# mbdriscoll/indigo

Hardware: AMD Instinct MI355X
Metric: SENSE AHA evals/sec (256^3 x 8-coil non-Cartesian) (higher is better)
Workload: dtype complex64 (f32)

## Files before the change

include/indigo_hip.h:

```cpp
#ifndef INDIGO_HIP_H
#define INDIGO_HIP_H

#include <stddef.h>
#include <stdint.h>

#ifdef __cplusplus
extern "C" {
#endif

#define IG_ABI_VERSION 1

#define IG_OK            0
#define IG_ERR_HIP       1
#define IG_ERR_ARG       2
#define IG_ERR_NODEVICE  3
#define IG_ERR_UNSUPPORTED 4
#define IG_ERR_NOMEM     5

#define IG_H2D 1
#define IG_D2H 2
#define IG_D2D 3

typedef struct ig_ctx   ig_ctx;
typedef struct ig_fft   ig_fft;
// ... 68 lines not shown
int  ig_csoft_c64(ig_ctx* ctx, int64_t n0, int64_t n1, int64_t n2, int64_t c0, int64_t c1, int64_t c2, int64_t ncols,
                  float tau, void* x, int64_t ldx);
int  ig_grad3_c64(ig_ctx* ctx, int64_t n0, int64_t n1, int64_t n2, int64_t ncols, const void* x, int64_t ldx,
                  float alpha_re, float alpha_im, float beta_re, float beta_im, void* y, int64_t ldy);
int  ig_grad3h_c64(ig_ctx* ctx, int64_t n0, int64_t n1, int64_t n2, int64_t ncols, const void* u, int64_t ldu,
                   float alpha_re, float alpha_im, float beta_re, float beta_im, void* y, int64_t ldy);
int  ig_tv_dual_c64(ig_ctx* ctx, int64_t n0, int64_t n1, int64_t n2, int64_t ncols, const void* xn, int64_t ldxn,
                    const void* xo, int64_t ldxo, float sigma, float mu, void* u, int64_t ldu);
int  ig_grad4_c64(ig_ctx* ctx, int64_t n0, int64_t n1, int64_t n2, int64_t nt, const void* x, int64_t ldx,
                  float alpha_re, float alpha_im, float beta_re, float beta_im, void* y, int64_t ldy);
int  ig_grad4h_c64(ig_ctx* ctx, int64_t n0, int64_t n1, int64_t n2, int64_t nt, const void* u, int64_t ldu,
                   float alpha_re, float alpha_im, float beta_re, float beta_im, void* y, int64_t ldy);
int  ig_tv4_dual_c64(ig_ctx* ctx, int64_t n0, int64_t n1, int64_t n2, int64_t nt, const void* xn, int64_t ldxn,
                     const void* xo, int64_t ldxo, float sigma, float mu, float mu_t, void* u, int64_t ldu);
int  ig_llr_svt_c64(ig_ctx* ctx, int64_t n0, int64_t n1, int64_t n2, int64_t nt, int64_t b0, int64_t b1, int64_t b2,
                    int64_t s0, int64_t s1, int64_t s2, float tau, void* x, int64_t ldx);
int  ig_llr_nuc_c64(ig_ctx* ctx, int64_t n0, int64_t n1, int64_t n2, int64_t nt, int64_t b0, int64_t b1, int64_t b2,
                    int64_t s0, int64_t s1, int64_t s2, const void* x, int64_t ldx, float* nuc);
int  ig_basis_c64(ig_ctx* ctx, int64_t n, int64_t nk, int64_t nt, const void* phi, int64_t ldphi, int adjoint,
                  const void* x, int64_t ldx, float alpha_re, float alpha_im, float beta_re, float beta_im,
                  void* y, int64_t ldy);
int  ig_psf_mix_c64(ig_ctx* ctx, int64_t n, int64_t nc, int64_t nk, const float* kern, const void* x, int64_t ldx,
                    void* y, int64_t ldy, int64_t sg, int64_t sc);
int  ig_coil_maps_c64(ig_ctx* ctx, int64_t n, int64_t nc, int64_t nm, const void* maps, int adjoint, const void* x,
                      float alpha_re, float alpha_im, float beta_re, float beta_im, void* y, int64_t ldi, int64_t sg, int64_t sc);

int  ig_ccsrmm(ig_ctx* ctx, int adjoint, int exwrite,
               int64_t M, int64_t K, int64_t N, int64_t nnz,
               float alpha_re, float alpha_im,
               const void* vals, const int32_t* colind, const int32_t* rowptr,
               const void* X, int64_t ldx,
               float beta_re, float beta_im,
               void* Y, int64_t ldy);

int  ig_ccsrmm_t(ig_ctx* ctx,
                 int64_t M, int64_t K, int64_t N, int64_t nnz,
                 float alpha_re, float alpha_im,
                 const void* vals_t, const int32_t* colind_t, const int32_t* rowptr_t,
                 const void* X, int64_t ldx,
                 float beta_re, float beta_im,
                 void* Y, int64_t ldy);

int  ig_ccsrmm_t_grid(ig_ctx* ctx,
                      int64_t M, int64_t K, int64_t N, int64_t nnz,
                      float alpha_re, float alpha_im,
                      const void* vals_t, const int32_t* colind_t, const int32_t* rowptr_t,
                      const void* X, int64_t ldx,
                      float beta_re, float beta_im,
                      void* Y, int64_t ldy,
                      const int16_t* support, int64_t n0, int64_t nm, const int32_t* xrow_perm);

int  ig_ccsrmm_il(ig_ctx* ctx,
                  int64_t M, int64_t K, int64_t N, int64_t nnz,
                  float alpha_re, float alpha_im,
                  const void* vals, const int32_t* colind, const int32_t* rowptr,
                  const void* X_il,
                  float beta_re, float beta_im,
                  void* Y, int64_t ldy);
int  ig_ccsrmm_il_rw(ig_ctx* ctx,
                     int64_t M, int64_t K, int64_t N, int64_t nnz,
                     float alpha_re, float alpha_im,
                     const void* vals, const float* vals_re, const int32_t* colind, const int32_t* rowptr,
                     const void* X_il,
                     float beta_re, float beta_im,
                     void* Y, int64_t ldy);
int  ig_ccsrmm_t_grid_il(ig_ctx* ctx,
                         int64_t M, int64_t K, int64_t N, int64_t nnz,
                         float alpha_re, float alpha_im,
                         const void* vals_t, const int32_t* colind_t, const int32_t* rowptr_t,
                         const void* X, int64_t ldx,
                         void* Y_il,
                         const int16_t* support, int64_t n0, int64_t nm);

int  ig_grid_bricks_count(int64_t M, const int32_t* rowptr, const int32_t* colind, int64_t n0, int64_t nm, int64_t ns,
                          int bm, int bs, int unit, int32_t* brick_entries);
int  ig_grid_bricks_fill(int64_t M, const int32_t* rowptr, const int32_t* colind, const void* vals, int64_t n0, int64_t nm,
                         int64_t ns, int bm, int bs, int unit, const int64_t* brick_ptr, void* entries,
                         uint32_t* round_rows);
int  ig_ccsrmm_t_bricks(ig_ctx* ctx, int64_t M, int64_t K, int64_t N, float alpha_re, float alpha_im,
                        const void* entries, const uint32_t* round_rows, const void* X, int64_t ldx, void* Y_il,
                        const int16_t* support, int64_t n0, int64_t nm, int bm, int bs, const int32_t* tasks, int64_t ntasks,
                        const int32_t* brick_table, const int32_t* shared_bricks, int64_t nshared, int support_tile, int support_zwords,
                        int entry_words);

int  ig_grid_slots_build(int64_t nbricks, const int64_t* brick_ptr, const void* entries12, const uint32_t* entry_rows, int ncell,
                         void* entries16, int32_t* brick_slots, int32_t* slot_ptr, int64_t* nslots);
int  ig_ccsrmm_t_slots(ig_ctx* ctx, int64_t M, int64_t K, int64_t N, float alpha_re, float alpha_im,
                       const void* entries16, const int32_t* slot_ptr, const void* X, int64_t ldx, void* Y_il,
                       const int16_t* support, int64_t n0, int64_t nm, int bm, int bs, const int32_t* tasks, int64_t ntasks,
                       const int32_t* brick_table, const int32_t* shared_bricks, int64_t nshared, int support_tile, int support_zwords,
                       int entry_words );

int  ig_grid_gather_sep(ig_ctx* ctx, int64_t M, int64_t NC, int tw, const void* records, int64_t rec_stride, const void* X_il,
                        int64_t n0, int64_t nm, int64_t ns, float alpha_re, float alpha_im, float beta_re, float beta_im,
                        void* Y, int64_t ldy, const uint32_t* group_order);
int  ig_grid_gather_sep_group(int64_t NC, int tw);

int  ig_grid_shares_count(int64_t M, const uint32_t* records, int tw, int64_t n0, int64_t nm, int64_t ns, int bm, int bs, int32_t* brick_shares);
int  ig_grid_shares_fill(int64_t M, const uint32_t* records, int tw, int64_t n0, int64_t nm, int64_t ns, int bm, int bs,
                         const int64_t* brick_ptr, uint32_t* shares);
int  ig_grid_scatter_sep(ig_ctx* ctx, int64_t M, int64_t NC, int tw, void* records, int64_t rec_stride, const void* shares, const void* X, int64_t ldx,
                         void* Y_il, int64_t n0, int64_t nm, int64_t ns, int bm, int bs, const int32_t* tasks, int64_t ntasks,
                         const int32_t* brick_table, const int32_t* shared_table, int64_t nshared, int support_tile,
                         float alpha_re, float alpha_im);

int  ig_ccsrmm_t_bricks_wide(ig_ctx* ctx, int64_t M, int64_t K, float alpha_re, float alpha_im,
                             const void* entries, const uint32_t* entry_rows, const void* X, int64_t ldx, void* Y, int64_t ldy,
                             const int32_t* tasks, int64_t ntasks, const int32_t* brick_table, const uint32_t* owned_tiles);
int  ig_ccsrmm_t_bricks_wide_grid(ig_ctx* ctx, int64_t M, int64_t K, float alpha_re, float alpha_im,
                                  const void* entries, const uint32_t* entry_rows, const void* X, int64_t ldx, void* Y, int64_t ldy,
                                  const int32_t* tasks, int64_t ntasks, const int32_t* brick_table, const uint32_t* owned_tiles,
                                  int64_t n0, int64_t nm, int bm, int bs,
                                  int entry_words );

int  ig_ccsrmm_rowperm(ig_ctx* ctx, int64_t M, int64_t K, int64_t N, int64_t nnz,
                       float alpha_re, float alpha_im,
                       const void* vals, const int32_t* colind, const int32_t* rowptr,
                       const void* X, int64_t ldx,
                       float beta_re, float beta_im,
                       void* Y, int64_t ldy,
                       const int32_t* yrow_perm);

int  ig_ccsrmm_xrows(ig_ctx* ctx, int64_t M, int64_t K, int64_t N, int64_t nnz,
                     float alpha_re, float alpha_im,
                     const void* vals, const int32_t* colind_c, const int32_t* rowptr,
                     const void* X, int64_t ldx,
                     float beta_re, float beta_im,
                     void* Y, int64_t ldy,
                     const int32_t* xrows, int64_t nxrows);

int  ig_csr_runs_build(int64_t M, int64_t K, const int32_t* rowptr, const int32_t* colind, const void* vals,
                       int32_t* run_dptr, uint32_t* dcols, void* entries, int* all_real);
int  ig_ccsrmm_xrows_runs(ig_ctx* ctx, int64_t M, int64_t K, int64_t nnz, float alpha_re, float alpha_im, const int32_t* rowptr,
                          const int32_t* run_dptr, const uint32_t* dcols, const void* entries, int all_real,
                          const int32_t* run_order ,
                          const void* X, int64_t ldx, float beta_re, float beta_im, void* Y, int64_t ldy,
                          const int32_t* xrows, int64_t nxrows);

int  ig_csr_inspect(const int32_t* rowptr, const int32_t* colind, int64_t M, int64_t K,
                    int64_t* nzrow, int64_t* nzcol, int* exwrite);

int  ig_csr_transpose(int64_t M, int64_t K, int64_t nnz,
                      const int32_t* rowptr, const int32_t* colind, const void* vals,
                      int32_t* rowptr_t, int32_t* colind_t, void* vals_t);

int  ig_conemm(ig_ctx* ctx, int64_t M, int64_t K, int64_t N, float alpha_re, float alpha_im,
               const void* X, int64_t ldx, float beta_re, float beta_im, void* Y, int64_t ldy);
int  ig_cdiamm(ig_ctx* ctx, int adjoint, int64_t M, int64_t K, int64_t N, int64_t ndiag, const int32_t* offsets,
               const void* data, int64_t ld_data, float alpha_re, float alpha_im, const void* X, int64_t ldx,
               float beta_re, float beta_im, void* Y, int64_t ldy);
int  ig_cgemm(ig_ctx* ctx, int adjoint, int right, int64_t rows_m, int64_t cols_m, int64_t p,
              float alpha_re, float alpha_im, const void* M, int64_t ldm, const void* X, int64_t ldx,
              float beta_re, float beta_im, void* Y, int64_t ldy);

int  ig_interp3_count(int64_t m, const int64_t* N, double width, const double* coord, int32_t* rowptr);
int  ig_interp3_fill(int64_t m, const int64_t* N, double width, const double* table, int64_t ntable,
                     const double* coord, const int32_t* rowptr, int32_t* colind, float* weights, int grid_order);
int  ig_interp3_fill_modulated(int64_t m, const int64_t* N, double width, const double* table, int64_t ntable,
                               const double* coord, const int32_t* rowptr, int32_t* colind, void* values, int grid_order,
                               const double* phase_x, const double* phase_y, const double* phase_z, double scale);
int  ig_interp3_sep_words(int tw);
int  ig_interp3_sep(int64_t m, const int64_t* N, double width, const double* table, int64_t ntable, const double* coord,
                    int grid_order, const double* sign_x, const double* sign_y, const double* sign_z, double scale,
                    int tw, uint32_t* records);
int  ig_grid_support(int64_t nnz, const int32_t* colind, int64_t n0, int64_t n1, int64_t n2, int tile, int zw_in, int zw_out, int16_t* table);

int  ig_fft_plan(ig_ctx* ctx, int rank, const int64_t* dims, int64_t batch,
                 ig_fft** plan, size_t* workspace_bytes);
int  ig_fft_exec(ig_fft* plan, const void* x, void* y, int direction ,
                 void* workspace );
int  ig_fft_describe(ig_fft* plan, char* buf, size_t len);
int  ig_fft_inplace_workspace(ig_fft* plan, size_t* bytes);

int  ig_fft_plan_padded(ig_ctx* ctx, const int64_t* dims, const int64_t* box_lo, const int64_t* box_dims,
                        int64_t batch, int grid_layout, ig_fft** plan, size_t* workspace_bytes);
int  ig_fft_set_support_tile(ig_fft* plan, int tile);
int  ig_fft_set_axis_shift(ig_fft* plan, int axis, int64_t shift);
int64_t ig_fft_zc_size(const int64_t* dims, const int64_t* box_dims, int64_t coils, int64_t piece_bytes);
int64_t ig_fft_zc_offset(const int64_t* dims, const int64_t* box_dims, int64_t coils, int64_t piece_bytes, int64_t kx, int64_t ky, int64_t z, int64_t coil);
int  ig_fft_support_words(int64_t n2, int* zw_in, int* zw_out);
int  ig_fft_padded_axis_kind(int64_t n, int* kind);
int  ig_fft_exec_padded(ig_fft* plan, const void* x, int64_t x_bstride, const void* w, void* y, void* workspace,
                        const int16_t* support);
int  ig_fft_exec_cropped(ig_fft* plan, const void* y, const void* w, void* x, int64_t x_bstride, void* workspace,
                         const int16_t* support);
int  ig_fft_exec_cropped_sum(ig_fft* plan, const void* y, const void* w, void* x, void* workspace,
                             const int16_t* support);
// ... 25 lines not shown
```

indigo_amd/_lib.py:

```python
import ctypes
import os
import sys
from ctypes import (POINTER, c_char_p, c_double, c_float, c_int, c_int32, c_int64,
                    c_size_t, c_void_p)

_HERE = os.path.dirname(os.path.abspath(__file__))
_LIB = None

IG_OK = 0
IG_H2D, IG_D2H, IG_D2D = 1, 2, 3

PROTOTYPES = {
    "ig_abi_version":     (c_int, []),
    "ig_device_count":    (c_int, [POINTER(c_int)]),
    "ig_init":            (c_int, [c_int, POINTER(c_void_p)]),
    "ig_init_on_stream":  (c_int, [c_int, c_void_p, POINTER(c_void_p)]),
    "ig_destroy":         (None,  [c_void_p]),
    "ig_last_error":      (c_char_p, [c_void_p]),
    "ig_sync":            (c_int, [c_void_p]),
    "ig_stream":          (c_void_p, [c_void_p]),
    "ig_device_name":     (c_int, [c_void_p, c_char_p, c_size_t]),
    "ig_mem_info":        (c_int, [c_void_p, POINTER(c_size_t), POINTER(c_size_t)]),
    "ig_set_option":      (c_int, [c_void_p, c_char_p, c_int64]),
    "ig_library_bytes":   (c_int, [c_void_p, POINTER(c_size_t)]),
    "ig_malloc":          (c_int, [c_void_p, c_size_t, POINTER(c_void_p)]),
    "ig_free":            (c_int, [c_void_p, c_void_p]),
    "ig_probe_placement": (c_int, [c_void_p, c_void_p, c_size_t, POINTER(c_double)]),
    "ig_memset0":         (c_int, [c_void_p, c_void_p, c_size_t]),
    "ig_copy2d":          (c_int, [c_void_p, c_void_p, c_size_t, c_void_p, c_size_t, c_size_t, c_size_t, c_int]),
    "ig_event_create":    (c_int, [c_void_p, POINTER(c_void_p)]),
    "ig_event_record":    (c_int, [c_void_p]),
    "ig_event_elapsed_ms": (c_int, [c_void_p, c_void_p, POINTER(c_float)]),
    "ig_event_destroy":   (c_int, [c_void_p]),
    "ig_graph_begin":     (c_int, [c_void_p]),
    "ig_graph_end":       (c_int, [c_void_p, POINTER(c_void_p)]),
    "ig_graph_abort":     (c_int, [c_void_p]),
    "ig_graph_launch":    (c_int, [c_void_p]),
    "ig_graph_destroy":   (c_int, [c_void_p]),
    "ig_prof_enable":     (c_int, [c_void_p, c_int]),
    "ig_prof_report":     (c_int, [c_void_p, c_char_p, c_size_t]),
    "ig_caxpby":          (c_int, [c_void_p, c_int64, c_float, c_float, c_void_p, c_float, c_float, c_void_p]),
    "ig_cscal":           (c_int, [c_void_p, c_int64, c_float, c_float, c_void_p]),
    "ig_cdotc":           (c_int, [c_void_p, c_int64, c_void_p, c_void_p, POINTER(c_double)]),
    "ig_scnrm2sq":        (c_int, [c_void_p, c_int64, c_void_p, POINTER(c_double)]),
    "ig_cmax":            (c_int, [c_void_p, c_int64, c_float, c_void_p]),
    "ig_scalars":         (c_int, [c_void_p, POINTER(c_void_p), POINTER(c_int)]),
    "ig_cdotc_dev":       (c_int, [c_void_p, c_int64, c_void_p, c_void_p, c_void_p]),
    "ig_scnrm2sq_dev":    (c_int, [c_void_p, c_int64, c_void_p, c_void_p]),
    "ig_scalar_ratio":    (c_int, [c_void_p, c_void_p, c_void_p, c_void_p, c_double]),
    "ig_scalar_ratio_gated": (c_int, [c_void_p, c_void_p, c_void_p, c_void_p, c_double, c_void_p, c_void_p, c_double]),
    "ig_scalar_copy":     (c_int, [c_void_p, c_void_p, c_void_p, c_int64]),
    "ig_scalar_read":     (c_int, [c_void_p, c_void_p, c_int64, c_void_p]),
    "ig_cg_dot":          (c_int, [c_void_p, c_int64, c_void_p, c_void_p, c_float]),
    "ig_cg_step_r":       (c_int, [c_void_p, c_int64, c_void_p, c_void_p, c_void_p, c_void_p, c_double, c_void_p]),
    "ig_cg_step_xp":      (c_int, [c_void_p, c_int64, c_void_p, c_void_p, c_void_p, c_void_p, c_void_p, c_void_p, c_void_p, c_void_p]),
    "ig_caxpby_dev":      (c_int, [c_void_p, c_int64, c_void_p, c_float, c_void_p, c_void_p, c_float, c_void_p]),
    "ig_csum_cols":       (c_int, [c_void_p, c_int64, c_int64, c_void_p, c_int64, c_float, c_float, c_float, c_float, c_void_p]),
    "ig_csum_il":         (c_int, [c_void_p, c_int64, c_int64, c_void_p, c_float, c_float, c_float, c_float, c_void_p]),
    "ig_permute3_c64":    (c_int, [c_void_p, c_int64, c_int64, c_int64, c_void_p, c_int64, c_void_p, c_int64,
                                   c_float, c_float, c_float, c_float, c_void_p, c_int64]),
    "ig_dwt3_c64":        (c_int, [c_void_p, c_int64, c_int64, c_int64, c_int, c_int, c_int, c_int64, c_void_p, c_int64,
                                   c_float, c_float, c_float, c_float, c_void_p, c_int64]),
    "ig_csoft_c64":       (c_int, [c_void_p, c_int64, c_int64, c_int64, c_int64, c_int64, c_int64, c_int64, c_float,
                                   c_void_p, c_int64]),
    "ig_grad3_c64":       (c_int, [c_void_p, c_int64, c_int64, c_int64, c_int64, c_void_p, c_int64,
                                   c_float, c_float, c_float, c_float, c_void_p, c_int64]),
    "ig_grad3h_c64":      (c_int, [c_void_p, c_int64, c_int64, c_int64, c_int64, c_void_p, c_int64,
                                   c_float, c_float, c_float, c_float, c_void_p, c_int64]),
    "ig_tv_dual_c64":     (c_int, [c_void_p, c_int64, c_int64, c_int64, c_int64, c_void_p, c_int64, c_void_p, c_int64,
                                   c_float, c_float, c_void_p, c_int64]),
    "ig_grad4_c64":       (c_int, [c_void_p, c_int64, c_int64, c_int64, c_int64, c_void_p, c_int64,
                                   c_float, c_float, c_float, c_float, c_void_p, c_int64]),
    "ig_grad4h_c64":      (c_int, [c_void_p, c_int64, c_int64, c_int64, c_int64, c_void_p, c_int64,
                                   c_float, c_float, c_float, c_float, c_void_p, c_int64]),
    "ig_tv4_dual_c64":    (c_int, [c_void_p, c_int64, c_int64, c_int64, c_int64, c_void_p, c_int64, c_void_p, c_int64,
                                   c_float, c_float, c_float, c_void_p, c_int64]),
    "ig_llr_svt_c64":     (c_int, [c_void_p, c_int64, c_int64, c_int64, c_int64, c_int64, c_int64, c_int64, c_int64, c_int64, c_int64,
                                   c_float, c_void_p, c_int64]),
    "ig_llr_nuc_c64":     (c_int, [c_void_p, c_int64, c_int64, c_int64, c_int64, c_int64, c_int64, c_int64, c_int64, c_int64, c_int64,
                                   c_void_p, c_int64, c_void_p]),
    "ig_basis_c64":       (c_int, [c_void_p, c_int64, c_int64, c_int64, c_void_p, c_int64, c_int, c_void_p, c_int64,
                                   c_float, c_float, c_float, c_float, c_void_p, c_int64]),
    "ig_psf_mix_c64":     (c_int, [c_void_p, c_int64, c_int64, c_int64, c_void_p, c_void_p, c_int64, c_void_p, c_int64, c_int64, c_int64]),
    "ig_coil_maps_c64":   (c_int, [c_void_p, c_int64, c_int64, c_int64, c_void_p, c_int, c_void_p,
                                   c_float, c_float, c_float, c_float, c_void_p, c_int64, c_int64, c_int64]),
    "ig_ccsrmm_il":      (c_int, [c_void_p, c_int64, c_int64, c_int64, c_int64,
                                   c_float, c_float, c_void_p, c_void_p, c_void_p,
                                   c_void_p, c_float, c_float, c_void_p, c_int64]),
    "ig_ccsrmm_il_rw":    (c_int, [c_void_p, c_int64, c_int64, c_int64, c_int64,
                                   c_float, c_float, c_void_p, c_void_p, c_void_p, c_void_p,
                                   c_void_p, c_float, c_float, c_void_p, c_int64]),
    "ig_ccsrmm_t_grid_il": (c_int, [c_void_p, c_int64, c_int64, c_int64, c_int64,
                                    c_float, c_float, c_void_p, c_void_p, c_void_p,
                                    c_void_p, c_int64, c_void_p,
                                    c_void_p, c_int64, c_int64]),
    "ig_grid_bricks_count": (c_int, [c_int64, c_void_p, c_void_p, c_int64, c_int64, c_int64, c_int, c_int, c_int, c_void_p]),
    "ig_grid_bricks_fill": (c_int, [c_int64, c_void_p, c_void_p, c_void_p, c_int64, c_int64, c_int64, c_int, c_int, c_int, c_void_p, c_void_p, c_void_p]),
    "ig_ccsrmm_t_bricks": (c_int, [c_void_p, c_int64, c_int64, c_int64, c_float, c_float, c_void_p, c_void_p,
                                   c_void_p, c_int64, c_void_p, c_void_p, c_int64, c_int64, c_int, c_int, c_void_p, c_int64,
                                   c_void_p, c_void_p, c_int64, c_int, c_int, c_int]),
    "ig_ccsrmm":          (c_int, [c_void_p, c_int, c_int, c_int64, c_int64, c_int64, c_int64,
                                   c_float, c_float, c_void_p, c_void_p, c_void_p,
                                   c_void_p, c_int64, c_float, c_float, c_void_p, c_int64]),
    "ig_ccsrmm_t":        (c_int, [c_void_p, c_int64, c_int64, c_int64, c_int64,
                                   c_float, c_float, c_void_p, c_void_p, c_void_p,
                                   c_void_p, c_int64, c_float, c_float, c_void_p, c_int64]),
    "ig_ccsrmm_t_grid":   (c_int, [c_void_p, c_int64, c_int64, c_int64, c_int64,
                                   c_float, c_float, c_void_p, c_void_p, c_void_p,
                                   c_void_p, c_int64, c_float, c_float, c_void_p, c_int64,
                                   c_void_p, c_int64, c_int64, c_void_p]),
    "ig_grid_slots_build": (c_int, [c_int64, c_void_p, c_void_p, c_void_p, c_int, c_void_p, c_void_p, c_void_p, POINTER(c_int64)]),
    "ig_ccsrmm_t_slots":  (c_int, [c_void_p, c_int64, c_int64, c_int64, c_float, c_float, c_void_p, c_void_p, c_void_p, c_int64, c_void_p,
                                   c_void_p, c_int64, c_int64, c_int, c_int, c_void_p, c_int64, c_void_p, c_void_p, c_int64, c_int, c_int, c_int]),
    "ig_ccsrmm_t_bricks_wide": (c_int, [c_void_p, c_int64, c_int64, c_float, c_float, c_void_p, c_void_p, c_void_p, c_int64, c_void_p, c_int64,
                                        c_void_p, c_int64, c_void_p, c_void_p]),
    "ig_ccsrmm_t_bricks_wide_grid": (c_int, [c_void_p, c_int64, c_int64, c_float, c_float, c_void_p, c_void_p, c_void_p, c_int64, c_void_p, c_int64,
                                             c_void_p, c_int64, c_void_p, c_void_p, c_int64, c_int64, c_int, c_int, c_int]),
    "ig_fft_set_support_tile": (c_int, [c_void_p, c_int]),
    "ig_fft_set_axis_shift": (c_int, [c_void_p, c_int, c_int64]),
    "ig_csr_runs_build":  (c_int, [c_int64, c_int64, c_void_p, c_void_p, c_void_p, c_void_p, c_void_p, c_void_p, POINTER(c_int)]),
    "ig_ccsrmm_xrows_runs": (c_int, [c_void_p, c_int64, c_int64, c_int64, c_float, c_float, c_void_p, c_void_p, c_void_p, c_void_p, c_int, c_void_p,
                                     c_void_p, c_int64, c_float, c_float, c_void_p, c_int64, c_void_p, c_int64]),
    "ig_ccsrmm_xrows":    (c_int, [c_void_p, c_int64, c_int64, c_int64, c_int64,
                                   c_float, c_float, c_void_p, c_void_p, c_void_p,
                                   c_void_p, c_int64, c_float, c_float, c_void_p, c_int64, c_void_p, c_int64]),
    "ig_ccsrmm_rowperm":  (c_int, [c_void_p, c_int64, c_int64, c_int64, c_int64,
                                   c_float, c_float, c_void_p, c_void_p, c_void_p,
                                   c_void_p, c_int64, c_float, c_float, c_void_p, c_int64, c_void_p]),
    "ig_csr_inspect":     (c_int, [c_void_p, c_void_p, c_int64, c_int64,
                                   POINTER(c_int64), POINTER(c_int64), POINTER(c_int)]),
    "ig_csr_transpose":   (c_int, [c_int64, c_int64, c_int64, c_void_p, c_void_p, c_void_p,
                                   c_void_p, c_void_p, c_void_p]),
    "ig_conemm":          (c_int, [c_void_p, c_int64, c_int64, c_int64, c_float, c_float, c_void_p, c_int64, c_float, c_float, c_void_p, c_int64]),
    "ig_cdiamm":          (c_int, [c_void_p, c_int, c_int64, c_int64, c_int64, c_int64, c_void_p, c_void_p, c_int64,
                                   c_float, c_float, c_void_p, c_int64, c_float, c_float, c_void_p, c_int64]),
    "ig_cgemm":           (c_int, [c_void_p, c_int, c_int, c_int64, c_int64, c_int64, c_float, c_float, c_void_p, c_int64,
                                   c_void_p, c_int64, c_float, c_float, c_void_p, c_int64]),
    "ig_interp3_count":   (c_int, [c_int64, POINTER(c_int64), c_double, c_void_p, c_void_p]),
    "ig_interp3_fill":    (c_int, [c_int64, POINTER(c_int64), c_double, c_void_p, c_int64, c_void_p, c_void_p, c_void_p, c_void_p, c_int]),
    "ig_grid_support":    (c_int, [c_int64, c_void_p, c_int64, c_int64, c_int64, c_int, c_int, c_int, c_void_p]),
    "ig_fft_support_words": (c_int, [c_int64, POINTER(c_int), POINTER(c_int)]),
    "ig_fft_padded_axis_kind": (c_int, [c_int64, POINTER(c_int)]),
    "ig_fft_zc_size":     (c_int64, [POINTER(c_int64), POINTER(c_int64), c_int64, c_int64]),
    "ig_fft_zc_offset":   (c_int64, [POINTER(c_int64), POINTER(c_int64), c_int64, c_int64, c_int64, c_int64, c_int64, c_int64]),
    "ig_interp3_sep_words": (c_int, [c_int]),
    "ig_interp3_sep":     (c_int, [c_int64, POINTER(c_int64), c_double, c_void_p, c_int64, c_void_p, c_int, c_void_p, c_void_p, c_void_p, c_double,
                                   c_int, c_void_p]),
    "ig_grid_gather_sep": (c_int, [c_void_p, c_int64, c_int64, c_int, c_void_p, c_int64, c_void_p, c_int64, c_int64, c_int64, c_float, c_float, c_float, c_float,
                                   c_void_p, c_int64, c_void_p]),
    "ig_grid_gather_sep_group": (c_int, [c_int64, c_int]),
    "ig_grid_shares_count": (c_int, [c_int64, c_void_p, c_int, c_int64, c_int64, c_int64, c_int, c_int, c_void_p]),
    "ig_grid_shares_fill": (c_int, [c_int64, c_void_p, c_int, c_int64, c_int64, c_int64, c_int, c_int, c_void_p, c_void_p]),
    "ig_grid_scatter_sep": (c_int, [c_void_p, c_int64, c_int64, c_int, c_void_p, c_int64, c_void_p, c_void_p, c_int64, c_void_p, c_int64, c_int64, c_int64,
                                    c_int, c_int, c_void_p, c_int64, c_void_p, c_void_p, c_int64, c_int, c_float, c_float]),
    "ig_interp3_fill_modulated": (c_int, [c_int64, POINTER(c_int64), c_double, c_void_p, c_int64, c_void_p, c_void_p, c_void_p, c_void_p, c_int,
                                          c_void_p, c_void_p, c_void_p, c_double]),
    "ig_fft_plan":        (c_int, [c_void_p, c_int, POINTER(c_int64), c_int64, POINTER(c_void_p), POINTER(c_size_t)]),
    "ig_fft_exec":        (c_int, [c_void_p, c_void_p, c_void_p, c_int, c_void_p]),
    "ig_fft_describe":    (c_int, [c_void_p, c_char_p, c_size_t]),
    "ig_fft_inplace_workspace": (c_int, [c_void_p, POINTER(c_size_t)]),
    "ig_fft_destroy":     (c_int, [c_void_p]),
    "ig_fft_plan_padded": (c_int, [c_void_p, POINTER(c_int64), POINTER(c_int64), POINTER(c_int64), c_int64, c_int,
                                   POINTER(c_void_p), POINTER(c_size_t)]),
    "ig_fft_exec_padded": (c_int, [c_void_p, c_void_p, c_int64, c_void_p, c_void_p, c_void_p, c_void_p]),
    "ig_fft_exec_cropped": (c_int, [c_void_p, c_void_p, c_void_p, c_void_p, c_int64, c_void_p, c_void_p]),
    "ig_fft_exec_cropped_sum": (c_int, [c_void_p, c_void_p, c_void_p, c_void_p, c_void_p, c_void_p]),
    "ig_fft_exec_cropped_sum_slab": (c_int, [c_void_p, c_void_p, c_void_p, c_void_p, c_void_p, c_void_p, c_int, c_int64, c_int64]),
    "ig_fft_exec_cropped_slab": (c_int, [c_void_p, c_void_p, c_void_p, c_void_p, c_int64, c_void_p, c_void_p, c_int, c_int64, c_int64]),
    "ig_comm_preflight":  (c_int, []),
    "ig_comm_unique_id":  (c_int, [c_void_p]),
    "ig_comm_init_rank":  (c_int, [c_void_p, c_int, c_int, c_void_p, POINTER(c_void_p)]),
    "ig_comm_init_direct": (c_int, [c_void_p, c_int, c_int, c_char_p, c_size_t, c_double, POINTER(c_void_p)]),
    "ig_comm_info":       (c_int, [c_void_p, POINTER(c_int), POINTER(c_int), c_char_p, c_size_t]),
    "ig_allreduce_sum_f32": (c_int, [c_void_p, c_void_p, c_int64]),
    "ig_allreduce_sum_f32_side": (c_int, [c_void_p, c_void_p, c_int64]),
    "ig_comm_join":       (c_int, [c_void_p]),
    "ig_allreduce_max_f64_host": (c_int, [c_void_p, POINTER(c_double)]),
    "ig_allreduce_sum_f64_host": (c_int, [c_void_p, POINTER(c_double)]),
    "ig_comm_barrier":    (c_int, [c_void_p]),
    "ig_comm_destroy":    (c_int, [c_void_p]),
}


def lib_path():
    return os.environ.get("INDIGO_HIP_LIB") or os.path.join(_HERE, "lib", "libindigo_hip.so")


def lib():
    global _LIB
    if _LIB is not None:
        return _LIB
    path = lib_path()
    if not os.path.exists(path):
        raise RuntimeError(
            "indigo_amd: %s not found. Build it with `python -m indigo_amd.build` "
            "(needs hipcc); there is no CPU fallback." % path)
    if os.environ.get("INDIGO_HIP_WITH_TORCH", "0") == "1" and "torch" not in sys.modules:
        import torch
    handle = ctypes.CDLL(path)
    for name, (res, args) in PROTOTYPES.items():
        fn = getattr(handle, name)
        fn.restype = res
        fn.argtypes = args
    if handle.ig_abi_version() != 1:
        raise RuntimeError("indigo_amd: ABI version mismatch in %s" % path)
    _LIB = handle
    return _LIB


def last_error(ctx=None):
    msg = lib().ig_last_error(ctx)
    return msg.decode("utf-8", "replace") if msg else ""


def cplx(v):
    v = complex(v)
    return ctypes.c_float(v.real), ctypes.c_float(v.imag)


def check(rc, ctx=None, what=""):
    if rc != IG_OK:
        raise RuntimeError("%s failed (status %d): %s" % (what or "libindigo_hip call", rc, last_error(ctx)))


def device_count():
    n = c_int(0)
    lib().ig_device_count(ctypes.byref(n))
    return n.value
```

indigo_amd/analyses.py:

```python
from contextlib import contextmanager

import numpy as np

from indigo_amd.transforms import Visitor
from indigo_amd import operators as op


class Memusage(Visitor):

    def measure(self, node, ncols=1):
        self._seen = set()
        self._base = 0
        self._live = [0]
        self._cols = [ncols]
        self._peak = 0
        self.visit(node)
        return self._base + self._peak

    @contextmanager
    def _push(self, stack, value):
        stack.append(value)
        try:
            yield
        finally:
            stack.pop()

    def _ncols(self):
        return int(np.prod(self._cols, dtype=np.int64))

    def _round(self, nbytes):
        return nbytes

    def visit(self, node):
        self._peak = max(self._peak, sum(self._live))
        if isinstance(node, op.ZpadFFTMaps) and id(node) not in self._seen:
            self._seen.add(id(node))
            self._base += node.maps_bytes()
        if isinstance(node, (op.Product, op.UnscaledFFT, op.ZpadFFT, op.HeadRows)):
            with self._push(self._live, self._round(node._mem_usage(self._ncols()))):
                self._peak = max(self._peak, sum(self._live))
                self.generic_visit(node)
        elif isinstance(node, op.ToeplitzNormal):
            if id(node) not in self._seen:
                self._seen.add(id(node))
                self._base += node.kernel_bytes()
            with self._push(self._live, self._round(node._mem_usage(self._ncols()))):
                self._peak = max(self._peak, sum(self._live))
        elif isinstance(node, op.Kron) and isinstance(node.left, op.Eye):
            with self._push(self._cols, node.left.shape[0]):
                self.visit(node.right)
        elif isinstance(node, op.SpMatrix):
            if id(node) not in self._seen:
                self._seen.add(id(node))
                self._base += (node.shape[0] + 1) * 4 + node.nnz * 4 + node.nnz * 8
        elif isinstance(node, (op.DenseMatrix, op.FrameBasis, op.CoilMaps)):
            if id(node) not in self._seen:
                self._seen.add(id(node))
                self._base += node._matrix.nbytes
        else:
            self.generic_visit(node)


class ScratchUsage(Memusage):

    def measure(self, node, ncols=1):
        super().measure(node, ncols)
        return self._peak // 8

    def _round(self, nbytes):
        elems = (nbytes + 7) // 8
        return (elems + 31) // 32 * 32 * 8


class TreeHasOp(Visitor):
    def __init__(self, op_classes):
        self._op_classes = tuple(op_classes)

    def search(self, node):
        self._found = False
        self.visit(node)
        return self._found

    def visit(self, node):
        if isinstance(node, self._op_classes):
            self._found = True
        self.generic_visit(node)
```

indigo_amd/backends/backend.py:

```python
import logging
from contextlib import contextmanager

import numpy as np
import scipy.sparse as spp

import indigo_amd.operators as op

log = logging.getLogger(__name__)
_C64 = np.dtype('complex64')


WAVELETS = {
    'haar': (2 ** -0.5, 2 ** -0.5),
    'db2': (0.48296291314453416, 0.8365163037378079, 0.22414386804201339, -0.12940952255126037),
    'db4': (0.23037781330889645, 0.7148465705529156, 0.630880767929859, -0.027983769416859594,
            -0.18703481171909306, 0.03084138183556063, 0.032883011666885176, -0.010597401785069018),
}
WAVELET_IDS = {'haar': 0, 'db2': 1, 'db4': 2}
DWT_MAX_AXIS = 1024


def dwt_plan(dims, wavelet, levels):
    taps = len(WAVELETS[wavelet])
    c = [int(n) for n in dims]
# ... 154 lines not shown
                return None
            dup = self._backend.zero_array(self.shape, self.dtype, name=name)
            dup._copy(self)
            return dup

        @classmethod
        def to_device(cls, backend, arr, name=''):
            arr_f = np.require(arr, requirements='F')
            d_arr = cls(backend, arr.shape, arr.dtype, name=name)
            d_arr.copy_from(arr_f)
            return d_arr

        def __setitem__(self, slc, other):
            assert isinstance(slc, slice) and not (slc.start or slc.stop), "dndarray setitem cant slice"
            self._copy(other)

        def __del__(self):
            if getattr(self, '_own', False) and hasattr(self, '_arr'):
                self._memory.pop(id(self), None)
                try:
                    self._free()
                except Exception:
                    pass

        def __getitem__(self, slc):
            raise NotImplementedError()

        def _copy_from(self, arr):
            raise NotImplementedError()

        def _copy_to(self, arr):
            raise NotImplementedError()

        def _copy(self, d_arr):
            raise NotImplementedError()

        def _malloc(self, shape, dtype):
            raise NotImplementedError()

        def _free(self):
            raise NotImplementedError()

        def _zero(self):
            raise NotImplementedError()

    def copy_array(self, arr, name=''):
        return self.dndarray.to_device(self, arr, name=name)

    def empty_array(self, shape, dtype, name=''):
        return self.dndarray(self, shape, dtype, name=name)

    def zero_array(self, shape, dtype, name=''):
        d_arr = self.empty_array(shape, dtype, name=name)
        d_arr._zero()
        return d_arr

    def zeros_like(self, other, name=''):
        return self.zero_array(other.shape, other.dtype, name=name)

    def rand_array(self, shape, dtype=_C64, name='', seed=None):
        rng = np.random.default_rng(seed)
        x = rng.random(shape) + 1j * rng.random(shape)
        x = np.require(x, dtype=_C64, requirements='F')
        return self.copy_array(x, name=name)

    def get_max_threads(self):
        return 1

    def barrier(self):
        pass

    def mem_usage(self):
        total = 0
        rows = []
        for name, shape, dtype in list(self.dndarray._memory.values()):
            n = int(np.prod(shape, dtype=np.int64)) * dtype.itemsize
            rows.append((n, name, shape, dtype))
            total += n
        log.info("Memory report:")
        for n, name, shape, dtype in sorted(rows, key=lambda r: r[0]):
            if n > 1e6:
                log.info("  %40s: % 3.0f MB, %20s, %15s", name, n / 1e6, shape, dtype)
        return total

    def reserve_scratch(self, nelems):
        self._scratch = self.empty_array((max(int(nelems), 1),), _C64, name='scratch')
        self._scratch_pos = 0

    @contextmanager
    def scratch(self, shape=None, nbytes=None):
        assert not (shape is not None and nbytes is not None), \
            "Specify either shape or nbytes to backend.scratch()."
        if nbytes is not None:
            shape = (int(nbytes) // _C64.itemsize,)
        size = int(np.prod(shape, dtype=np.int64))
        arena = getattr(self, '_scratch', None)
        if arena is not None and self._scratch_pos + size > arena.size:
            log.warning("scratch arena too small (wanted %d elements at offset %d of %d); allocating dynamically",
                        size, self._scratch_pos, arena.size)
            arena = None
        if arena is not None:
            pos = self._scratch_pos
            mem = arena[pos:pos + size].reshape(tuple(shape))
            bump = (size + 31) // 32 * 32
            self._scratch_pos += bump
            try:
                yield mem
            finally:
                self._scratch_pos -= bump
        else:
            mem = self.zero_array(tuple(shape), dtype=_C64, name='scratch(dynamic)')
            yield mem
            del mem

    def SpMatrix(self, M=None, **kwargs):
        assert (M is not None and spp.issparse(M)) or kwargs.get('struct') is not None
        return op.SpMatrix(self, M, **kwargs)

    def DenseMatrix(self, M, **kwargs):
        assert isinstance(M, np.ndarray) and M.ndim == 2
        return op.DenseMatrix(self, M, **kwargs)

    def Diag(self, v, **kwargs):
        v = np.require(v, requirements='F')
        if v.ndim > 1:
            v = v.flatten(order='A')
        dtype = kwargs.pop('dtype', _C64)
        if np.dtype(dtype) == _C64:
            from indigo_amd.structured import DiagS
            return self.SpMatrix(struct=DiagS(v.size, [('vec', v.astype(_C64))]), **kwargs)
        return self.SpMatrix(spp.diags(v, offsets=0).astype(dtype), **kwargs)

    def Adjoint(self, A, **kwargs):
        return op.Adjoint(self, A, **kwargs)

    def KronI(self, c, B, **kwargs):
        return op.Kron(self, self.Eye(c), B, **kwargs)

    def Kron(self, A, B, **kwargs):
        return op.Kron(self, A, B, **kwargs)

    def BlockDiag(self, Ms, **kwargs):
        return op.BlockDiag(self, *Ms, **kwargs)

    def VStack(self, Ms, **kwargs):
        return op.VStack(self, *Ms, **kwargs)

    def HStack(self, Ms, **kwargs):
        return op.HStack(self, *Ms, **kwargs)

    def UnscaledFFT(self, shape, dtype=_C64, **kwargs):
        return op.UnscaledFFT(self, shape, dtype=dtype, **kwargs)

    def Eye(self, n, dtype=_C64, **kwargs):
        return op.Eye(self, n, dtype=dtype, **kwargs)

    def ZpadFFT(self, grid_shape, box_shape, weights, **kwargs):
        return op.ZpadFFT(self, grid_shape, box_shape, weights, **kwargs)

    def One(self, shape, dtype=_C64, **kwargs):
        return op.One(self, shape, dtype=dtype, **kwargs)

    def FFT(self, shape, dtype=_C64, **kwargs):
        n = int(np.prod(shape))
        if np.dtype(dtype) == _C64:
            from indigo_amd.structured import DiagS
            c = (np.ones(1, dtype=dtype) / np.sqrt(n))[0]
            return self.SpMatrix(struct=DiagS(n, [('const', c)]), name='scale') * self.UnscaledFFT(shape, dtype, **kwargs)
        s = np.ones(n, order='F', dtype=dtype) / np.sqrt(n)
        return self.Diag(s, name='scale') * self.UnscaledFFT(shape, dtype, **kwargs)

    @staticmethod
    def fftc_mod_phases(ft_shape):
        return [(np.arange(n) - (n // 2) / 2.0) * ((n // 2) / n) for n in ft_shape]

    @staticmethod
    def fftc_mod(ft_shape, dtype=_C64):
        phase = 0
        for i, ph in enumerate(Backend.fftc_mod_phases(ft_shape)):
            phase = phase + ph.reshape([-1 if j == i else 1 for j in range(len(ft_shape))])
        return np.exp(1j * 2.0 * np.pi * phase).astype(dtype)

    def FFTc(self, ft_shape, dtype=_C64, normalize=True, **kwargs):
        if np.dtype(dtype) == _C64:
            from indigo_amd.structured import DiagS, SepPhase
            M = self.SpMatrix(struct=DiagS(int(np.prod(ft_shape)), [('sep', SepPhase(ft_shape, self.fftc_mod_phases(ft_shape)))]), name='mod')
        else:
            M = self.Diag(self.fftc_mod(ft_shape, dtype), name='mod')
        F = self.FFT(ft_shape, dtype=dtype, **kwargs) if normalize else self.UnscaledFFT(ft_shape, dtype=dtype, **kwargs)
        return M * F * M

    @staticmethod
    def zpad_rows(M, N, mode='center'):
        if mode == 'center':
            slc = tuple(slice(m // 2 + int(np.ceil(-n / 2)), m // 2 + int(np.ceil(n / 2))) for m, n in zip(M, N))
        elif mode == 'edge':
            slc = tuple(slice(n) for n in N)
        else:
            raise ValueError("unknown zpad mode %r" % mode)
        x = np.arange(int(np.prod(M)), dtype=np.int64).reshape(M, order='F')
        return x[slc].flatten(order='F')

    def Zpad(self, M, N, mode='center', dtype=_C64, **kwargs):
        rows = self.zpad_rows(M, N, mode)
        cols = np.arange(rows.size)
        if np.dtype(dtype) == _C64:
            from indigo_amd.structured import SelectS
            return self.SpMatrix(struct=SelectS((int(np.prod(M)), int(np.prod(N))), rows, cols, np.ones(rows.size, dtype=_C64)), **kwargs)
        mat = spp.coo_matrix((np.ones(rows.size), (rows, cols)), shape=(int(np.prod(M)), int(np.prod(N))), dtype=dtype)
        return self.SpMatrix(mat, **kwargs)

    def Crop(self, M, N, dtype=_C64, **kwargs):
        return self.Zpad(N, M, dtype=dtype, **kwargs).H

    def AxisPermute(self, dims, perm, **kwargs):
        return op.AxisPermute(self, dims, perm, **kwargs)

# ... 297 lines not shown
        w = int(width) if (interleaved and width is not None) else C
        K2 = kern.size // n
        K = int(round(np.sqrt(K2)))
        assert n >= 1 and C >= 1 and w >= C and K * K * n == kern.size, (kern.shape, n)
        rows = n * w
        assert x.size == rows * K and y.size == rows * K, (x.shape, y.shape, n, w, K)
        P = self.psf_unpack(kern.to_host(), n, K)
        shape = (w, n, K) if interleaved else (n, w, K)
        v = x.to_host().reshape(shape, order='F').astype(np.complex128)
        out = y.to_host().reshape(shape, order='F').copy()
        if interleaved:
            out[:C] = np.einsum('gab,cgb->cga', P, v[:C]).astype(_C64)
        else:
            out[:] = np.einsum('gab,gcb->gca', P, v).astype(_C64)
        y.copy_from(np.asfortranarray(out.reshape(y.shape, order='F')))

    def ToeplitzNormal(self, dims, maps, kern, K, **kwargs):
        return op.ToeplitzNormal(self, dims, maps, kern, K, **kwargs)

    def supports_padded_fft(self, grid, ncoils=None):
        return False

    def ccsrmm(self, y, A_shape, A_indx, A_ptr, A_vals, x, alpha=1, beta=0, adjoint=False, exwrite=False):
        raise NotImplementedError()

    def cdiamm(self, y, shape, offsets, data, x, alpha=1.0, beta=0.0, adjoint=True):
        raise NotImplementedError()

    def onemm(self, y, x, alpha=1, beta=0):
        raise NotImplementedError()

    def cgemm(self, y, M, x, alpha, beta, forward):
        raise NotImplementedError()

    def csymm(self, y, M, x, alpha, beta, left=True):
        raise NotImplementedError()

    def max(self, val, arr):
        raise NotImplementedError()

    def inspect(self, csr):
        counts = np.bincount(csr.indices, minlength=csr.shape[1])
        nzrow = int(np.count_nonzero(np.diff(csr.indptr)))
        return nzrow, int(np.count_nonzero(counts)), bool(counts.max(initial=0) <= 1)

    class csr_matrix(object):
        _index_base = 0

        def __init__(self, backend, A, name='mat'):
            if not spp.isspmatrix_csr(A):
                A = A.tocsr()
            A = self._type_correct(A)
            assert A.nnz < 2 ** 31 and max(A.shape) < 2 ** 31, "int32 CSR indices"
            self._backend = backend
            self._name = name
            self.shape = tuple(int(s) for s in A.shape)
            self.dtype = A.dtype
            self.rowPtrs = backend.copy_array(A.indptr.astype(np.int32) + self._index_base, name=name + ".rowPtrs")
            self.colInds = backend.copy_array(A.indices.astype(np.int32) + self._index_base, name=name + ".colInds")
            self.values = backend.copy_array(A.data, name=name + ".data")
            nzrow, nzcol, self._exwrite = backend.inspect(A)
            self._row_frac = nzrow / A.shape[0] if A.shape[0] else 1.0
            self._col_frac = nzcol / A.shape[1] if A.shape[1] else 1.0
            self._grid_il = False

        @staticmethod
        def _check_panels(y, x, vals):
            assert x.dtype == _C64, "Bad dtype: expected complex64, got %s" % x.dtype
            assert y.dtype == _C64, "Bad dtype: expected complex64, got %s" % y.dtype
            assert vals.dtype == _C64

        def forward(self, y, x, alpha=1, beta=0):
            self._check_panels(y, x, self.values)
            il = {'x_il': True} if self._grid_il else {}
            self._backend.ccsrmm(y, self.shape, self.colInds, self.rowPtrs, self.values,
                                 x, alpha=alpha, beta=beta, adjoint=False, exwrite=True, **il)

        def adjoint(self, y, x, alpha=1, beta=0):
            self._check_panels(y, x, self.values)
            il = {'y_il': True} if self._grid_il else {}
            self._backend.ccsrmm(y, self.shape, self.colInds, self.rowPtrs, self.values,
                                 x, alpha=alpha, beta=beta, adjoint=True, exwrite=self._exwrite, **il)

        def set_grid_interleaved(self, flag=True):
            self._grid_il = bool(flag)

        def set_grid_support(self, table, n0, nm, zw=16):
            pass

        def set_grid_bricks(self, n0, nm, ns, ncols=8, bm=2, bs=2, chunk=4096, run=4096):
            pass

        def set_row_order(self, perm):
            pass

        @property
        def nbytes(self):
            return self.rowPtrs.nbytes + self.colInds.nbytes + self.values.nbytes

        @property
        def nnz(self):
            return self.values.size

        def _type_correct(self, A):
            return A.astype(_C64)

    class dia_matrix(object):

        def __init__(self, backend, A, name='mat'):
            assert isinstance(A, spp.dia_matrix)
            A = A.astype(_C64)
            self._backend = backend
            self.data = backend.copy_array(np.asfortranarray(A.data.T), name=name + ".data")
            self.offsets = backend.copy_array(A.offsets.astype(np.int32), name=name + ".offsets")
            self.shape = tuple(int(s) for s in A.shape)
            self.dtype = A.dtype
            self._row_frac = 1
            self._col_frac = 1
            self._exwrite = False

        def forward(self, y, x, alpha=1, beta=0):
            self._backend.cdiamm(y, self.shape, self.offsets, self.data, x, alpha=alpha, beta=beta, adjoint=False)

        def adjoint(self, y, x, alpha=1, beta=0):
            self._backend.cdiamm(y, self.shape, self.offsets, self.data, x, alpha=alpha, beta=beta, adjoint=True)

        @property
        def nbytes(self):
            return self.offsets.nbytes + self.data.nbytes

        @property
        def nnz(self):
            return self.data.size

    def cg(self, A, b_h, x_h, lamda=0.0, tol=1e-10, maxiter=100, team=None):
        in_place = isinstance(x_h, self.dndarray)
        x = x_h if in_place else self.copy_array(x_h, name='x')
        resid = b_h.copy(name='b') if isinstance(b_h, self.dndarray) else self.copy_array(b_h, name='b')
        q = x.copy()

        def shifted(dst, src):
            A.eval(dst, src)
            if lamda:
                self.axpby(1, dst, lamda, src)

        shifted(q, x)
        self.axpby(1, resid, -1, q)
        d = resid.copy(name='p')
        rho = rho0 = self.pnorm2(resid, team)
        trail = []
        for it in range(maxiter):
            shifted(q, d)
            step = rho / self.pdot(d, q, team)
            self.axpby(1, x, step, d)
            self.axpby(1, resid, -step, q)
            rho, rho_old = self.pnorm2(resid, team), rho
            self.axpby(rho / rho_old, d, 1, resid)
            trail.append(float(np.sqrt(rho / rho0)))
            log.info("iter %d, residual %g", it, trail[-1])
            if trail[-1] < tol:
                log.info("cg reached tolerance")
                break
        else:
            log.info("cg reached maxiter")
        if not in_place:
            x.copy_to(x_h)
# ... 62 lines not shown
```

indigo_amd/backends/hip.py:

```python
import ctypes
import logging
import os

import numpy as np

from indigo_amd import _lib
from indigo_amd._lib import cplx as _cplx
from indigo_amd.backends.backend import WAVELET_IDS, Backend
from indigo_amd.grid_formats import brick_tasks, weights_are_real

log = logging.getLogger(__name__)
_C64 = np.dtype('complex64')


class HipBackend(Backend):

    def __init__(self, device_id=0, stream=None):
        super().__init__(device_id)
        self._L = _lib.lib()
        ctx = ctypes.c_void_p()
        if stream is None:
            rc = self._L.ig_init(int(device_id), ctypes.byref(ctx))
        else:
            rc = self._L.ig_init_on_stream(int(device_id), ctypes.c_void_p(stream), ctypes.byref(ctx))
        _lib.check(rc, None, "ig_init")
        self._ctx = ctx
        self.device_id = int(device_id)
        self._plans = dict()
        self.adjoint_policy = 'transpose'
        self._placement_log = []
        self.tuning = dict(placement_candidates=3, placement_min_bytes=1 << 31, placement_window_gb=24, placement_window_allocs=3, fold_odd_axes=True, real_gridding=True, gather_order=True, cg_graph=False, bricks=(4, 8), slots=(1, 2), slot_shape=(4, 4, 256, 64), support_tile={8: 4, 4: 8}, brick_shape={8: (2, 2, 4096, 4096), 4: (2, 4, 4096, 4096)}, xrows=True, runs=True, wide_bricks=True,
                           wide_brick_shape=(2, 2), wide_task_shape=(8192, 2048),
                           separable=True, sep_gather=True, sep_scatter=True, shares=(4, 8), shares_min_tw=6, share_shape={8: (4, 4, 128, 1024), 4: (4, 4, 128, 1024)})

    def __del__(self):
        try:
            for entry in getattr(self, '_plans', {}).values():
                self._L.ig_fft_destroy(entry[0])
            if getattr(self, '_ctx', None):
                self._L.ig_destroy(self._ctx)
                self._ctx = None
        except Exception:
            pass

    def _check(self, rc, what):
        if rc != 0:
            _lib.check(rc, self._ctx, what)

    def barrier(self):
        self._check(self._L.ig_sync(self._ctx), "ig_sync")

    @property
    def stream(self):
        return self._L.ig_stream(self._ctx) or 0

    def device_name(self):
        buf = ctypes.create_string_buffer(256)
        self._check(self._L.ig_device_name(self._ctx, buf, 256), "ig_device_name")
        return buf.value.decode()

    def set_option(self, name, value):
        self._check(self._L.ig_set_option(self._ctx, name.encode(), int(value)), "ig_set_option(%s)" % name)
        for entry in self._plans.values():
            self._L.ig_fft_destroy(entry[0])
        self._plans = dict()

    def mem_usage(self):
        own = ctypes.c_size_t()
        self._check(self._L.ig_library_bytes(self._ctx, ctypes.byref(own)), "ig_library_bytes")
        return super().mem_usage() + own.value

    def mem_info(self):
        free, total = ctypes.c_size_t(), ctypes.c_size_t()
        self._check(self._L.ig_mem_info(self._ctx, ctypes.byref(free), ctypes.byref(total)), "ig_mem_info")
        return free.value, total.value

    def event(self):
        ev = ctypes.c_void_p()
        self._check(self._L.ig_event_create(self._ctx, ctypes.byref(ev)), "ig_event_create")
        return ev

    def record(self, ev):
        self._check(self._L.ig_event_record(ev), "ig_event_record")

    def elapsed_ms(self, start, stop):
        ms = ctypes.c_float()
        self._check(self._L.ig_event_elapsed_ms(start, stop, ctypes.byref(ms)), "ig_event_elapsed_ms")
        return ms.value

    def event_destroy(self, ev):
        self._L.ig_event_destroy(ev)

    def profile(self, on=True):
        self._check(self._L.ig_prof_enable(self._ctx, 1 if on else 0), "ig_prof_enable")
        self._prof_on = bool(on)

    def profile_report(self):
        buf = ctypes.create_string_buffer(1 << 16)
        self._check(self._L.ig_prof_report(self._ctx, buf, len(buf)), "ig_prof_report")
        out = {}
        for line in buf.value.decode().splitlines():
            name, n, ms, nbytes = line.split()
            out[name] = dict(launches=int(n), total_ms=float(ms), avg_ms=float(ms) / max(int(n), 1), bytes=float(nbytes))
        return out

    class dndarray(Backend.dndarray):

        def _malloc(self, shape, dtype):
            b = self._backend
            if self.nbytes >= int(b.tuning.get('placement_min_bytes', 1 << 31)):
                slack = int(b.tuning.get('placement_window_gb', 0))
                if slack > 0:
                    ptr = self._malloc_window(slack)
                    if ptr is not None:
                        return ptr
                ncand = int(b.tuning.get('placement_candidates', 1))
                if ncand > 1:
                    return self._malloc_best_placed(ncand)
            ptr = ctypes.c_void_p()
            b._check(b._L.ig_malloc(b._ctx, self.nbytes, ctypes.byref(ptr)), "ig_malloc(%d bytes)" % self.nbytes)
            return ptr.value

        def _malloc_window(self, slack_gb):
            b = self._backend
            GBs = 1 << 30
            nalloc = max(1, int(b.tuning.get('placement_window_allocs', 3)))
            worst = b.tuning.get('placement_pick') == 'worst'
            cands = []
            try:
                for _ in range(nalloc):
                    free, total = ctypes.c_size_t(), ctypes.c_size_t()
                    need = (self.nbytes + (slack_gb + 4) * GBs) if not cands else 2 * (self.nbytes + slack_gb * GBs)
                    if b._L.ig_mem_info(b._ctx, ctypes.byref(free), ctypes.byref(total)) != 0 or free.value < need:
                        break
                    base = ctypes.c_void_p()
                    if b._L.ig_malloc(b._ctx, self.nbytes + slack_gb * GBs, ctypes.byref(base)) != 0:
                        break
                    cands.append([None, base.value, 0, []])
                    times = []
                    for off in range(slack_gb + 1):
                        ms = ctypes.c_double(0.0)
                        b._check(b._L.ig_probe_placement(b._ctx, ctypes.c_void_p(base.value + off * GBs), self.nbytes, ctypes.byref(ms)), "ig_probe_placement")
                        times.append(ms.value)
                    if len(cands) == 1:
# ... 767 lines not shown
```

indigo_amd/backends/hip_csr.py:

```python
import logging

import numpy as np

from indigo_amd import _lib, grid_formats
from indigo_amd._lib import cplx as _cplx
from indigo_amd.backends.backend import Backend

log = logging.getLogger(__name__)
_C64 = np.dtype('complex64')

_BRICK_ARRAYS = dict(tasks=".brickTasks", table=".brickTable", entries=".brickEntries", rounds=".brickRoundRows", shared=".sharedBricks")
_SLOT_ARRAYS = dict(tasks=".slotTasks", table=".slotTable", entries=".slotEntries", slot_ptr=".slotPtr", shared=".slotSharedBricks")
_SHARE_ARRAYS = dict(tasks=".shareTasks", table=".shareTable", shares=".shares", shared=".shareSharedBricks")
_WIDE_ARRAYS = dict(owned=".wideOwnedTiles", tasks=".wideTasks", table=".wideTable", entries=".wideEntries", rows=".wideEntryRows")
_RUN_ARRAYS = dict(order=".runOrder", dptr=".runPtr", dcols=".runCols", entries=".runEntries")


def _ptr(a):
    return None if a is None else a._arr


class csr_matrix(Backend.csr_matrix):

    def __init__(self, backend, A, name='mat'):
# ... 183 lines not shown
        if self._perm is None and 16 <= ncols <= 64 and self._col_frac <= 0.6 and self.values.size >= self.shape[1] and t['xrows']:
            sub = self._touched()
            return 'xrows_runs' if ncols == 64 and t.get('runs', True) and sub[0].size * 512 < 2 ** 32 and self._runs(sub) is not None else 'xrows'
        return 'csr' if self._perm is None else 'rowperm'

    def adjoint_route(self, ncols, beta, y):
        b, perm = self._backend, self._perm
        scatter = perm is None and beta == 0 and y.contiguous
        shf = self._format('_shares', ncols, exact=True)
        if shf is not None and scatter and self._grid_il and shf['ntasks'] > 0 and b.tuning.get('sep_scatter', True):
            return 'shares'
        br = self._format('_bricks', ncols, exact=True)
        if br is not None and scatter and self._grid_il and ncols == br['ncols']:
            return 'bricks'
        sl = self._format('_slots', ncols, exact=True)
        if sl is not None and scatter and ncols == sl['ncols'] and sl['ntasks'] > 0:
            return 'slots'
        if (ncols == 64 and beta == 0 and perm is None and not self._grid_il and self.shape[1] % 16 == 0
                and self.shape[1] > 0 and self.shape[0] * 512 < 2 ** 31 and self.values.size >= self.shape[1] // 4
                and b.tuning['wide_bricks'] and self._wide_bricks() is not None):
            return 'wide'
        if self._grid_il:
            assert scatter, "interleaved panels: no row order, beta = 0"
            return 'gather_il'
        if perm is not None:
            assert not self._exwrite and b.adjoint_policy == 'transpose' and ncols <= 8, \
                "row-ordered matrices use the packed transposed gather"
        if (self._gather_support() is not None or perm is not None) and not self._exwrite and b.adjoint_policy == 'transpose':
            return 'gather_t_grid'
        return 'scatter' if self._exwrite or b.adjoint_policy != 'transpose' else 'gather_t'

    def _gather_support(self):
        return self._support if self._support_zw == 16 else None

    def _scatter_support(self, ncols, y):
        fine = self._format('_support_fine', ncols)
        tab, tile = fine if fine is not None else (self._support[0] if self._support is not None else None, 16)
        if tab is None:
            y._zero()
        return tab, tile

    def _call(self, kernel, *args):
        b = self._backend
        b._check(getattr(b._L, kernel)(b._ctx, *args), kernel)

    def _fwd_sep(self, y, x, alpha, beta):
        sep = self._sep
        order = self._gather_order(x.shape[1]) if self._backend.tuning.get('gather_order', True) else None
        self._call("ig_grid_gather_sep", self.shape[0], x.shape[1], sep['tw'], sep['records']._arr, sep['stride'], x._arr, *sep['dims'],
                   *_cplx(complex(alpha) * sep['gconst']), *_cplx(beta), y._arr, y._leading_dim, _ptr(order))

    def _fwd_il_rw(self, y, x, alpha, beta):
        self._call("ig_ccsrmm_il_rw", *self.shape, x.shape[1], self.values.size, *_cplx(alpha), self.values._arr, self._real_values()._arr,
                   self.colInds._arr, self.rowPtrs._arr, x._arr, *_cplx(beta), y._arr, y._leading_dim)

    def _fwd_il(self, y, x, alpha, beta):
        self._call("ig_ccsrmm_il", *self.shape, x.shape[1], self.values.size, *_cplx(alpha), self.values._arr, self.colInds._arr,
                   self.rowPtrs._arr, x._arr, *_cplx(beta), y._arr, y._leading_dim)

    def _fwd_xrows_runs(self, y, x, alpha, beta):
        sub, runs = self._xrows, self._runs_fmt
        self._call("ig_ccsrmm_xrows_runs", *self.shape, self.values.size, *_cplx(alpha), self.rowPtrs._arr, runs['dptr']._arr, runs['dcols']._arr,
                   runs['entries']._arr, runs['all_real'], _ptr(runs['order']), x._arr, x._leading_dim, *_cplx(beta), y._arr, y._leading_dim,
                   sub[0]._arr, sub[0].size)

    def _fwd_xrows(self, y, x, alpha, beta):
        sub = self._xrows
        self._call("ig_ccsrmm_xrows", *self.shape, x.shape[1], self.values.size, *_cplx(alpha), self.values._arr, sub[1]._arr, self.rowPtrs._arr,
                   x._arr, x._leading_dim, *_cplx(beta), y._arr, y._leading_dim, sub[0]._arr, sub[0].size)

    def _fwd_rowperm(self, y, x, alpha, beta):
        self._call("ig_ccsrmm_rowperm", *self.shape, x.shape[1], self.values.size, *_cplx(alpha), self.values._arr, self.colInds._arr,
                   self.rowPtrs._arr, x._arr, x._leading_dim, *_cplx(beta), y._arr, y._leading_dim, self._perm._arr)

    _FORWARD = dict(sep=_fwd_sep, il_rw=_fwd_il_rw, il=_fwd_il, xrows_runs=_fwd_xrows_runs, xrows=_fwd_xrows, rowperm=_fwd_rowperm,
                    csr=Backend.csr_matrix.forward)

    def forward(self, y, x, alpha=1, beta=0):
        if self._grid_il:
            assert self._perm is None and x.contiguous, "interleaved panels: no row order, contiguous grid panel"
        self._check_panels(y, x, self.values)
        self._FORWARD[self.forward_route(x.shape[1])](self, y, x, alpha, beta)

    def _adj_shares(self, y, x, alpha, beta):
        sep, shf = self._sep, self._format('_shares', x.shape[1], exact=True)
        self._scatter_support(x.shape[1], y)
        self._call("ig_grid_scatter_sep", self.shape[0], x.shape[1], sep['tw'], sep['recx']._arr, sep['stride_x'], shf['shares']._arr, x._arr,
                   x._leading_dim, y._arr, *sep['dims'], shf['bm'], shf['bs'], shf['tasks']._arr, shf['ntasks'], shf['table']._arr,
                   shf['shared']._arr, shf['nshared'], shf['tile'], *_cplx(complex(alpha) * np.conj(sep['gconst'])))

    def _adj_bricks(self, y, x, alpha, beta, kernel="ig_ccsrmm_t_bricks", which='_bricks', rows='rounds'):
        f = self._format(which, x.shape[1], exact=True)
        tab, tile = self._scatter_support(x.shape[1], y)
        self._call(kernel, *self.shape, x.shape[1], *_cplx(alpha), f['entries']._arr, f[rows]._arr, x._arr, x._leading_dim, y._arr, _ptr(tab),
                   f['n0'], f['nm'], f['bm'], f['bs'], f['tasks']._arr, f['ntasks'], f['table']._arr, f['shared']._arr, f['nshared'], tile,
                   self._support_zw, f['words'])

    def _adj_slots(self, y, x, alpha, beta):
        self._adj_bricks(y, x, alpha, beta, "ig_ccsrmm_t_slots", '_slots', 'slot_ptr')

    def _adj_wide(self, y, x, alpha, beta):
        wb = self._wide
        self._call("ig_ccsrmm_t_bricks_wide_grid", *self.shape, *_cplx(alpha), wb['entries']._arr, wb['rows']._arr, x._arr, x._leading_dim, y._arr,
                   y._leading_dim, wb['tasks']._arr, wb['ntasks'], wb['table']._arr, wb['owned']._arr, *wb['geom'], wb['words'])

    def _adj_gather_il(self, y, x, alpha, beta):
        pt, it, dt = self._transposed()
        tab, n0, nm = self._gather_support() or (None, 0, 0)
        self._call("ig_ccsrmm_t_grid_il", *self.shape, x.shape[1], dt.size, *_cplx(alpha), dt._arr, it._arr, pt._arr, x._arr, x._leading_dim,
                   y._arr, _ptr(tab), n0, nm)

    def _adj_gather_t(self, y, x, alpha, beta):
        pt, it, dt = self._transposed()
        self._backend.ccsrmm_t(y, self.shape, it, pt, dt, x, alpha=alpha, beta=beta, support=self._gather_support(), xperm=self._perm)

    def _adj_scatter(self, y, x, alpha, beta):
        self._backend.ccsrmm(y, self.shape, self.colInds, self.rowPtrs, self.values, x, alpha=alpha, beta=beta, adjoint=True, exwrite=self._exwrite)

    _ADJOINT = dict(shares=_adj_shares, bricks=_adj_bricks, slots=_adj_slots, wide=_adj_wide, gather_il=_adj_gather_il,
                    gather_t_grid=_adj_gather_t, scatter=_adj_scatter, gather_t=_adj_gather_t)

    def adjoint(self, y, x, alpha=1, beta=0):
        self._check_panels(y, x, self.values)
        self._ADJOINT[self.adjoint_route(x.shape[1], beta, y)](self, y, x, alpha, beta)
```

indigo_amd/csrc/ig_gridsep.hip:

```cpp
#include "ig_common.h"
#include <vector>
#include <thread>
#include <atomic>
#include <algorithm>
#include <cstring>

namespace {

constexpr int BLK = 256;
constexpr int WPB = BLK / 64;

__device__ __forceinline__ int64_t xcd_block(int64_t b, int64_t nb) {
    const int64_t q = nb >> 3, rem = nb & 7;
    const int64_t xcd = b & 7, idx = b >> 3;
    return (xcd < rem) ? xcd * (q + 1) + idx : rem * (q + 1) + (xcd - rem) * q + idx;
}

__host__ __device__ constexpr int sep_words(int tw) { return tw == 4 ? 16 : 32; }

template <int NC, int TW, int NBT, int CG>
__device__ __forceinline__ void gather_rows(float4& acc, const float4* __restrict__ X4, const uint32_t (&offm)[TW], const float (&w1)[TW],
                                            const float (&w2)[TW], float w0, int j2, int c2, int ns, uint32_t plane, int nc2u) {
#pragma unroll
    for (int c0 = 0; c0 < TW; c0 += CG) {
        if (c0 >= nc2u) break;
        float4 v[CG][NBT];
#pragma unroll
        for (int g = 0; g < CG; ++g) {
            int cc = c0 + g;
            cc = cc < c2 ? cc : c2 - 1;
            int js = j2 + cc;
            if (js >= ns) js -= ns;
            const uint32_t offs = (uint32_t)js * plane;
#pragma unroll
            for (int b = 0; b < NBT; ++b) v[g][b] = X4[(size_t)(offs + offm[b])];
        }
#pragma unroll
        for (int g = 0; g < CG; ++g) {
            const float ws = (c0 + g < c2) ? w0 * w2[c0 + g < TW ? c0 + g : 0] : 0.f;
#pragma unroll
            for (int b = 0; b < NBT; ++b) {
                const float w = ws * w1[b];
                acc.x = fmaf(w, v[g][b].x, acc.x); acc.y = fmaf(w, v[g][b].y, acc.y);
                acc.z = fmaf(w, v[g][b].z, acc.z); acc.w = fmaf(w, v[g][b].w, acc.w);
            }
        }
    }
}

template <int NC, int TW, int BMODE>
__global__ void __launch_bounds__(BLK)
k_grid_gather_sep(int64_t M, const uint32_t* __restrict__ rec, int rs , const float4* __restrict__ X4, int n0, int nm, int ns,
                  float2* __restrict__ Y, int64_t ldy, float2 alpha, float2 beta, const uint32_t* __restrict__ order) {
    constexpr int QL = NC / 2, XL = TW <= 4 ? 4 : 8, LPS = QL * XL, SPW = 64 / LPS;
    constexpr int CG = TW <= 4 ? 4 : 2;
    static_assert(LPS <= 64 && NC >= 2, "a sample's lanes fit a wave");
    const int lane = threadIdx.x & 63;
    const int q = lane % QL, i = (lane / QL) % XL, g = lane / LPS;
    int64_t blk = xcd_block(blockIdx.x, gridDim.x);
    if (order) { const uint32_t o = order[blk]; blk = o < gridDim.x ? (int64_t)o : blk; }
    const int64_t wave = blk * WPB + (threadIdx.x >> 6);
    const int64_t t = wave * SPW + g;
    const bool ok = t < M;
    const uint32_t* __restrict__ r = rec + (size_t)(ok ? t : M - 1) * (uint32_t)rs;
    const uint32_t h0 = r[3 * TW], h1 = r[3 * TW + 1];
    const int j0 = (int)(h0 & 0xffffu), j1 = (int)(h0 >> 16), j2 = (int)(h1 & 0xffffu);
    const int c0 = (int)((h1 >> 16) & 15u), c1 = (int)((h1 >> 20) & 15u), c2 = (int)((h1 >> 24) & 15u);
    const int iv = i < c0 ? i : c0 - 1;
    const float w0 = (i < c0 && ok) ? __uint_as_float(r[iv]) : 0.f;
    float w1[TW], w2[TW];
#pragma unroll
    for (int b = 0; b < TW; ++b) { w1[b] = b < c1 ? __uint_as_float(r[TW + b]) : 0.f; w2[b] = __uint_as_float(r[2 * TW + b]); }
    int jx = j0 + iv;
    if (jx >= n0) jx -= n0;
    uint32_t offm[TW];
#pragma unroll
    for (int b = 0; b < TW; ++b) {
        int jm = j1 + (b < c1 ? b : c1 - 1);
        if (jm >= nm) jm -= nm;
        offm[b] = ((uint32_t)jm * (uint32_t)n0 + (uint32_t)jx) * QL + q;
    }
    const uint32_t plane = (uint32_t)nm * (uint32_t)n0 * QL;
    int nc2u = 1;
#pragma unroll
    for (int v = TW; v > 1; --v)
        if (__builtin_amdgcn_ballot_w64(c2 >= v)) { nc2u = v; break; }
    float4 acc = make_float4(0.f, 0.f, 0.f, 0.f);
    if (__builtin_amdgcn_ballot_w64(c1 >= TW)) gather_rows<NC, TW, TW, CG>(acc, X4, offm, w1, w2, w0, j2, c2, ns, plane, nc2u);
    else                                       gather_rows<NC, TW, TW - 1, CG>(acc, X4, offm, w1, w2, w0, j2, c2, ns, plane, nc2u);
#pragma unroll
    for (int off = QL; off < LPS; off <<= 1) {
        acc.x += __shfl_xor(acc.x, off, 64); acc.y += __shfl_xor(acc.y, off, 64);
        acc.z += __shfl_xor(acc.z, off, 64); acc.w += __shfl_xor(acc.w, off, 64);
    }
    if (i == 0 && ok) {
        float2* y0 = Y + (int64_t)(2 * q) * ldy + t;
        float2* y1 = y0 + ldy;
        float2 o0 = cmul(alpha, make_float2(acc.x, acc.y)), o1 = cmul(alpha, make_float2(acc.z, acc.w));
        if (BMODE == 1) { cfma(o0, beta, *y0); cfma(o1, beta, *y1); }
        *y0 = o0;
        *y1 = o1;
    }
}

struct ShareTask { int32_t lo, hi, bt, nb_flags; };
struct ShareBrick { int32_t brick, end; uint32_t mask_lo, mask_hi; };

typedef float v16f_t __attribute__((ext_vector_type(16)));

template <bool SHARED, int NG, int XW>
__device__ __forceinline__ void mfma_flush(v16f_t (&acc)[NG], float* __restrict__ Yf, int64_t pt, uint64_t mask, float2 alpha, float sgn_ai, bool f_ok,
                                           int beta, int mn, int n0, int nm, int bm, int bs, int st_log2) {
    const int xs_log2 = 4 - st_log2;
    const int xseg = (4 * beta) >> st_log2;
#pragma unroll
    for (int g = 0; g < NG; ++g) {
        if (g < bs) {
#pragma unroll
            for (int b = 0; b < 4; ++b) {
                if (b < bm) {
                    float* dst = Yf + (pt + 4 * beta + (int64_t)n0 * (b + (int64_t)nm * g)) * XW + mn;
                    const bool mine = f_ok && ((mask >> (xseg + ((b + bm * g) << xs_log2))) & 1ull);
                    float o[4];
#pragma unroll
                    for (int r = 0; r < 4; ++r) {
                        const float v = acc[g][4 * b + r];
                        const float pv = __int_as_float(__builtin_amdgcn_update_dpp(0, __float_as_int(v), 0xB1, 0xf, 0xf, false));
                        o[r] = fmaf(alpha.x, v, sgn_ai * pv);
                    }
                    if (mine) {
                        if (SHARED)
                            asm volatile("global_atomic_add_f32 %0, %1, off\n\tglobal_atomic_add_f32 %0, %2, off offset:%5\n\t"
                                         "global_atomic_add_f32 %0, %3, off offset:%6\n\tglobal_atomic_add_f32 %0, %4, off offset:%7"
                                         :: "v"(dst), "v"(o[0]), "v"(o[1]), "v"(o[2]), "v"(o[3]), "i"(XW * 4), "i"(2 * XW * 4), "i"(3 * XW * 4) : "memory");
                        else
                            asm volatile("global_store_dword %0, %1, off\n\tglobal_store_dword %0, %2, off offset:%5\n\t"
                                         "global_store_dword %0, %3, off offset:%6\n\tglobal_store_dword %0, %4, off offset:%7"
                                         :: "v"(dst), "v"(o[0]), "v"(o[1]), "v"(o[2]), "v"(o[3]), "i"(XW * 4), "i"(2 * XW * 4), "i"(3 * XW * 4) : "memory");
                    }
                    __builtin_amdgcn_sched_barrier(0);
                }
            }
        }
#pragma unroll
        for (int e = 0; e < 16; ++e) acc[g][e] = 0.f;
    }
}

template <int NC, int TW, int NG>
__global__ void __launch_bounds__(BLK, 3)
k_grid_scatter_mfma(const ShareTask* __restrict__ tasks, int ntasks, const ShareBrick* __restrict__ btab, const uint2* __restrict__ shares,
                    const uint32_t* __restrict__ recx, int rs ,
                    float* __restrict__ Yf, float2 alpha, int n0, int nm, int bm_log2, int bs_log2, int nbx, int nbm, int st_log2) {
    constexpr int RW = sep_words(TW), XW = 2 * NC, ZL = 3 * TW + 2;
    constexpr int PW = RW + 16;
    constexpr int G = 4, R = 16;
    static_assert(PW + TW + 6 <= 64 && XW <= 16 && NG == 4, "a ring slot holds record, panel row and the padded slow-axis weights");
    __shared__ uint32_t ring_all[WPB][R][64];
    __shared__ uint2 hdr_all[WPB][128];
    const int tid = threadIdx.x, lane = tid & 63;
    const int wv = __builtin_amdgcn_readfirstlane(tid >> 6);
    const int task = blockIdx.x * WPB + wv;
    if (task >= ntasks) return;
    const ShareTask tk = tasks[task];
    const int nb = tk.nb_flags & 0xffff;
    const bool shared = (tk.nb_flags >> 16) & 1;
    const int nsh = tk.hi - tk.lo;
    const int bm = 1 << bm_log2, bs = 1 << bs_log2;
    const int beta = lane >> 4, mn = lane & 15;
    uint32_t* __restrict__ ring = &ring_all[wv][0][0];

    int my_end = 0x7fffffff;
    uint32_t my_mlo = 0xffffffffu, my_mhi = 0xffffffffu;
    int64_t my_pt = 0;
    if (lane < nb) {
        const ShareBrick br = btab[tk.bt + lane];
        if (!shared) my_end = br.end - tk.lo;
        my_mlo = br.mask_lo; my_mhi = br.mask_hi;
        const int bx = br.brick % nbx, bmi = (br.brick / nbx) % nbm, bsi = br.brick / (nbx * nbm);
        my_pt = (int64_t)bx * 16 + (int64_t)n0 * (((int64_t)bmi << bm_log2) + (int64_t)nm * ((int64_t)bsi << bs_log2));
    }
    v16f_t acc[NG];
#pragma unroll
    for (int g = 0; g < NG; ++g)
// ... 18 lines not shown
    auto load_batch = [&](int b) __attribute__((always_inline)) {
        const int idx = b * 64 + lane;
        return idx < nsh ? shp[idx] : make_uint2(0u, 0u);
    };
    {
        const uint2 b0 = load_batch(0), b1 = load_batch(1);
        hdrs[lane] = b0;
        hdrs[64 + lane] = b1;
    }
    uint2 sh_next = load_batch(2);
    int cb = 0;

    auto request = [&](uint32_t (&w)[G], int gi) __attribute__((always_inline)) {
#pragma unroll
        for (int k = 0; k < G; ++k) {
            const int sraw = G * gi + k;
            const int sc = sraw < nsh ? sraw : nsh - 1;
            const uint32_t t = (uint32_t)__builtin_amdgcn_readfirstlane((int)hdrs[sc & 127].x) & 0x0fffffffu;
            w[k] = lane_base[(size_t)t * (uint32_t)rs];
        }
    };
    auto stage = [&](const uint32_t (&w)[G], int gi) __attribute__((always_inline)) {
#pragma unroll
        for (int k = 0; k < G; ++k) ring[((G * gi + k) & (R - 1)) * 64 + lane] = w[k];
    };
    auto process = [&](int gi) __attribute__((always_inline)) {
        for (int k = 0; k < G; ++k) {
            const int s = G * gi + k;
            if (s >= nsh) break;
            if (s >= cur_end) {
                int ph, pl; uint32_t mlo, mhi;
                brick_of(ph, pl, mlo, mhi);
                mfma_flush<false, NG, XW>(acc, Yf, ((int64_t)ph << 32) | (uint32_t)pl, ((uint64_t)mhi << 32) | mlo, alpha, sgn_ai, f_ok, beta, mn, n0, nm, bm, bs, st_log2);
                ++cur;
                cur_end = __builtin_amdgcn_readlane(my_end, cur & 63);
            }
            const uint2 hd = hdrs[s & 127];
            const uint32_t geo = (uint32_t)__builtin_amdgcn_readfirstlane((int)hd.y), gmask = (uint32_t)__builtin_amdgcn_readfirstlane((int)hd.x) >> 28;
            const char* slot = reinterpret_cast<const char*>(ring) + (s & (R - 1)) * 256;
            const int ox4 = (int)(geo & 31u) * 4 - 32, om4 = (int)((geo >> 5) & 31u) * 4 - 32, os4 = (int)((geo >> 10) & 31u) * 4 - 32;
            const unsigned dx = (unsigned)(mn4 - ox4), db = (unsigned)(beta4 - om4);
            const float ax = __uint_as_float(*reinterpret_cast<const uint32_t*>(slot + (dx < (unsigned)(4 * TW) ? dx : (unsigned)(4 * ZL))));
            const float wm = __uint_as_float(*reinterpret_cast<const uint32_t*>(slot + (db - 4u * TW < (unsigned)(4 * TW) ? db : (unsigned)(4 * ZL))));
            const float xv = __uint_as_float(*reinterpret_cast<const uint32_t*>(slot + xv_off));
            const uint32_t* wsp = reinterpret_cast<const uint32_t*>(slot + (PW + 3) * 4 - os4);
            const float bmx = wm * xv;
#pragma unroll
            for (int g = 0; g < NG; ++g)
                if ((gmask >> g) & 1u)
                    acc[g] = __builtin_amdgcn_mfma_f32_16x16x1f32(ax, bmx * __uint_as_float(wsp[g]), acc[g], 0, 0, 0);
        }
    };

    const int ngroups = (nsh + G - 1) / G;
    uint32_t wa[G], wb[G];
    request(wa, 0);
    request(wb, 1);
    stage(wa, 0);
    for (int gi = 0; gi < ngroups; gi += 2) {
        if (((G * gi) >> 6) != cb) {
            ++cb;
            hdrs[((cb + 1) & 1) * 64 + lane] = sh_next;
            sh_next = load_batch(cb + 2);
        }
        request(wa, gi + 2);
        process(gi);
        stage(wb, gi + 1);
        request(wb, gi + 3);
        process(gi + 1);
        stage(wa, gi + 2);
    }
    {
        int ph, pl; uint32_t mlo, mhi;
        brick_of(ph, pl, mlo, mhi);
        const int64_t pt = ((int64_t)ph << 32) | (uint32_t)pl;
        const uint64_t mask = ((uint64_t)mhi << 32) | mlo;
        if (shared) mfma_flush<true, NG, XW>(acc, Yf, pt, mask, alpha, sgn_ai, f_ok, beta, mn, n0, nm, bm, bs, st_log2);
        else        mfma_flush<false, NG, XW>(acc, Yf, pt, mask, alpha, sgn_ai, f_ok, beta, mn, n0, nm, bm, bs, st_log2);
    }
}

template <int NC>
__global__ void __launch_bounds__(BLK)
k_sep_pack_recx(int64_t rows, const float2* __restrict__ X, int64_t ld, float2* __restrict__ recx2 , int rs2 , int rw2 ) {
    for (int64_t e = (int64_t)blockIdx.x * BLK + threadIdx.x; e < rows * NC; e += (int64_t)gridDim.x * BLK)
        recx2[(e / NC) * rs2 + rw2 + e % NC] = X[(e % NC) * ld + e / NC];
}

template <int NC>
__global__ void __launch_bounds__(BLK)
k_grid_sep_zero(const ShareBrick* __restrict__ bricks, float4* __restrict__ Y4, int n0, int nm, int bm_log2, int bs_log2, int nbx, int nbm, int st_log2) {
    constexpr int QL = NC / 2, LR = 16 * QL;
    const ShareBrick br = bricks[blockIdx.x];
    const uint64_t mask = ((uint64_t)br.mask_hi << 32) | br.mask_lo;
    const int bx = br.brick % nbx, bmi = (br.brick / nbx) % nbm, bsi = br.brick / (nbx * nbm);
    const int64_t pt = (int64_t)bx * 16 + (int64_t)n0 * (((int64_t)bmi << bm_log2) + (int64_t)nm * ((int64_t)bsi << bs_log2));
    const int nrows = 1 << (bm_log2 + bs_log2), xs_log2 = 4 - st_log2;
    for (int e = threadIdx.x; e < nrows * LR; e += BLK) {
        const int row = e / LR, xq = e % LR, x = xq / QL;
        if ((mask >> ((x >> st_log2) + (row << xs_log2))) & 1ull) {
            const int im = row & ((1 << bm_log2) - 1), is = row >> bm_log2;
            Y4[(pt + (int64_t)n0 * (im + (int64_t)nm * is)) * QL + xq] = make_float4(0.f, 0.f, 0.f, 0.f);
        }
    }
}

struct ShareGeom { int64_t n[3]; int bdim[3]; int64_t nbr[3]; int tw, rw; };

struct AxisPiece { int brick, o, lo, hi; };
inline int axis_pieces(int j, int cnt, int64_t n, int bdim, AxisPiece* out) {
    int np = 0;
    int a = 0;
    while (a < cnt) {
        int64_t cell = j + a;
        if (cell >= n) cell -= n;
        const int brick = (int)(cell / bdim), off = (int)(cell % bdim);
        int run = bdim - off;
        if (run > cnt - a) run = cnt - a;
        if (cell + run > n) run = (int)(n - cell);
        out[np++] = AxisPiece{brick, off - a, a, a + run};
        a += run;
    }
    return np;
}

template <class F>
inline void for_shares(const ShareGeom& g, const uint32_t* r, F&& f) {
    const uint32_t h0 = r[3 * g.tw], h1 = r[3 * g.tw + 1];
    const int j[3] = {(int)(h0 & 0xffffu), (int)(h0 >> 16), (int)(h1 & 0xffffu)};
    const int cnt[3] = {(int)((h1 >> 16) & 15u), (int)((h1 >> 20) & 15u), (int)((h1 >> 24) & 15u)};
    AxisPiece px[9], pm[9], ps[9];
    const int nx = axis_pieces(j[0], cnt[0], g.n[0], g.bdim[0], px), nmm = axis_pieces(j[1], cnt[1], g.n[1], g.bdim[1], pm),
              nss = axis_pieces(j[2], cnt[2], g.n[2], g.bdim[2], ps);
    for (int c = 0; c < nss; ++c)
        for (int b = 0; b < nmm; ++b)
            for (int a = 0; a < nx; ++a) {
                const int64_t brick = px[a].brick + g.nbr[0] * (pm[b].brick + g.nbr[1] * (int64_t)ps[c].brick);
                const uint32_t geo = (uint32_t)(px[a].o + 8) | ((uint32_t)(pm[b].o + 8) << 5) | ((uint32_t)(ps[c].o + 8) << 10) |
                                     ((uint32_t)pm[b].lo << 15) | ((uint32_t)pm[b].hi << 18) | ((uint32_t)ps[c].lo << 22) | ((uint32_t)ps[c].hi << 25);
                const uint32_t gmask = g.bdim[2] <= 4 ? ((((1u << (ps[c].hi - ps[c].lo)) - 1u) << (ps[c].o + ps[c].lo)) & 15u) : 15u;
                f(brick, geo, gmask);
            }
}

inline int share_threads(int64_t M) {
    unsigned hw = std::thread::hardware_concurrency();
    int nt = (int)(hw ? hw : 4);
    if (nt > 16) nt = 16;
    if (M < 16384) nt = 1;
    return nt;
}

template <class F>
inline void run_threads(int nt, F&& body) {
    if (nt == 1) { body(0); return; }
    std::vector<std::thread> th;
    for (int t = 0; t < nt; ++t) th.emplace_back([t, &body]() { body(t); });
    for (auto& x : th) x.join();
}

inline bool share_geom(ShareGeom& g, int tw, int64_t n0, int64_t nm, int64_t ns, int bm, int bs) {
    auto pow2 = [](int v) { return v > 0 && (v & (v - 1)) == 0; };
    if (!(tw == 4 || tw == 6 || tw == 8) || n0 < 16 || n0 % 16 || nm < tw || ns < tw || !pow2(bm) || !pow2(bs) || bm > 16 || bs > 16 ||
        n0 > 65535 || nm > 65535 || ns > 65535)
        return false;
    g.n[0] = n0; g.n[1] = nm; g.n[2] = ns;
    g.bdim[0] = 16; g.bdim[1] = bm; g.bdim[2] = bs;
    g.nbr[0] = n0 / 16; g.nbr[1] = (nm + bm - 1) / bm; g.nbr[2] = (ns + bs - 1) / bs;
    g.tw = tw; g.rw = sep_words(tw);
    return g.nbr[0] * g.nbr[1] * g.nbr[2] < 0x7fffffffLL;
}

}

extern "C" {

int ig_grid_gather_sep_group(int64_t NC, int tw) {
    if (!(NC == 2 || NC == 4 || NC == 8) || !(tw == 4 || tw == 6 || tw == 8)) return 0;
    return WPB * (64 / ((int)(NC / 2) * (tw <= 4 ? 4 : 8)));
}

int ig_grid_gather_sep(ig_ctx* ctx, int64_t M, int64_t NC, int tw, const void* records, int64_t rec_stride, const void* X_il, int64_t n0, int64_t nm, int64_t ns,
                       float ar, float ai, float br, float bi, void* Y, int64_t ldy, const uint32_t* group_order) {
    IG_REQUIRE(ctx, ctx != nullptr, "ig_grid_gather_sep: ctx is NULL");
    IG_REQUIRE(ctx, M >= 0 && (NC == 2 || NC == 4 || NC == 8) && (tw == 4 || tw == 6 || tw == 8), "ig_grid_gather_sep: 2, 4 or 8 interleaved coils; tw 4, 6 or 8");
    IG_REQUIRE(ctx, n0 >= tw && nm >= tw && ns >= tw && n0 <= 65535 && nm <= 65535 && ns <= 65535 && n0 * nm * ns * (NC / 2) < (1LL << 32),
               "ig_grid_gather_sep: grid %lld x %lld x %lld x %lld coils out of range", (long long)n0, (long long)nm, (long long)ns, (long long)NC);
    IG_REQUIRE(ctx, M == 0 || (records && X_il && Y && ldy >= M), "ig_grid_gather_sep: NULL pointer or ldy < M");
    IG_REQUIRE(ctx, rec_stride >= sep_words(tw) && rec_stride % 4 == 0 && rec_stride <= 1024, "ig_grid_gather_sep: record stride %lld words", (long long)rec_stride);
    IG_REQUIRE(ctx, (reinterpret_cast<uintptr_t>(X_il) & 15u) == 0 && (reinterpret_cast<uintptr_t>(records) & 15u) == 0, "ig_grid_gather_sep: 16-byte aligned panel and records");
    if (M == 0) return IG_OK;
    if (int rc = ig_set_device(ctx)) return rc;
    const float2 alpha = make_float2(ar, ai), beta = make_float2(br, bi);
    const bool b0 = br == 0.f && bi == 0.f;
    ig_prof_scope prof(ctx, "grid_gather_sep");
#define IG_GS(NC_, TW_) do {                                                                                                     \
        constexpr int spw = 64 / ((NC_ / 2) * (TW_ <= 4 ? 4 : 8));                                                               \
        const int64_t blocks = ((M + spw - 1) / spw + WPB - 1) / WPB;                                                            \
        IG_REQUIRE(ctx, blocks <= 0x7fffffffLL, "ig_grid_gather_sep: too many samples for one launch");                          \
        if (b0) hipLaunchKernelGGL((k_grid_gather_sep<NC_, TW_, 0>), dim3((unsigned)blocks), dim3(BLK), 0, ctx->stream, M,       \
                                   (const uint32_t*)records, (int)rec_stride, (const float4*)X_il, (int)n0, (int)nm, (int)ns, (float2*)Y, ldy, alpha, beta, group_order); \
        else    hipLaunchKernelGGL((k_grid_gather_sep<NC_, TW_, 1>), dim3((unsigned)blocks), dim3(BLK), 0, ctx->stream, M,       \
                                   (const uint32_t*)records, (int)rec_stride, (const float4*)X_il, (int)n0, (int)nm, (int)ns, (float2*)Y, ldy, alpha, beta, group_order); \
    } while (0)
#define IG_GS_TW(NC_) do { if (tw == 4) IG_GS(NC_, 4); else if (tw == 6) IG_GS(NC_, 6); else IG_GS(NC_, 8); } while (0)
    if (NC == 8) IG_GS_TW(8);
    else if (NC == 4) IG_GS_TW(4);
    else IG_GS_TW(2);
#undef IG_GS_TW
#undef IG_GS
    IG_LAUNCH_CHECK(ctx, "k_grid_gather_sep");
    return IG_OK;
}


int ig_grid_shares_count(int64_t M, const uint32_t* records, int tw, int64_t n0, int64_t nm, int64_t ns, int bm, int bs, int32_t* brick_shares) {
    ShareGeom g;
    if (M < 0 || (M > 0 && !records) || !brick_shares || !share_geom(g, tw, n0, nm, ns, bm, bs))
        return ig_fail(nullptr, IG_ERR_ARG, "ig_grid_shares_count: a grid of a multiple of 16 points along x, bricks of 16 x bm x bs cells (powers of two <= 16); tw 4, 6 or 8");
    const int64_t nb = g.nbr[0] * g.nbr[1] * g.nbr[2];
    const int nt = share_threads(M);
    const int64_t per = (M + nt - 1) / nt;
    std::vector<std::vector<int32_t>> cnt((size_t)nt);
    std::atomic<int> bad{0};
    run_threads(nt, [&](int t) {
        cnt[t].assign((size_t)nb, 0);
        const int64_t lo = std::min<int64_t>(M, t * per), hi = std::min<int64_t>(M, lo + per);
        for (int64_t s = lo; s < hi; ++s)
            for_shares(g, records + (size_t)s * g.rw, [&](int64_t brick, uint32_t, uint32_t) { if (++cnt[t][brick] < 0) bad = 1; });
    });
    run_threads(nt, [&](int t) {
        const int64_t pb = (nb + nt - 1) / nt, lo = std::min<int64_t>(nb, t * pb), hi = std::min<int64_t>(nb, lo + pb);
        for (int64_t b = lo; b < hi; ++b) {
            int64_t sum = 0;
            for (int u = 0; u < nt; ++u) sum += cnt[u][b];
            if (sum > 0x7fffffffLL) { bad = 1; sum = 0; }
            brick_shares[b] = (int32_t)sum;
        }
    });
    if (bad) return ig_fail(nullptr, IG_ERR_ARG, "ig_grid_shares_count: a brick exceeds 2^31 shares");
    return IG_OK;
}

int ig_grid_shares_fill(int64_t M, const uint32_t* records, int tw, int64_t n0, int64_t nm, int64_t ns, int bm, int bs,
                        const int64_t* brick_ptr , uint32_t* shares ) {
    ShareGeom g;
    if (M < 0 || M >= (1LL << 28) || (M > 0 && (!records || !shares)) || !brick_ptr || !share_geom(g, tw, n0, nm, ns, bm, bs))
        return ig_fail(nullptr, IG_ERR_ARG, "ig_grid_shares_fill: bad arguments (fewer than 2^28 samples)");
    const int64_t nb = g.nbr[0] * g.nbr[1] * g.nbr[2];
    const int nt = share_threads(M);
    const int64_t per = (M + nt - 1) / nt;
    std::vector<std::vector<int32_t>> cur((size_t)nt);
    run_threads(nt, [&](int t) {
        cur[t].assign((size_t)nb, 0);
        const int64_t lo = std::min<int64_t>(M, t * per), hi = std::min<int64_t>(M, lo + per);
        for (int64_t s = lo; s < hi; ++s)
            for_shares(g, records + (size_t)s * g.rw, [&](int64_t brick, uint32_t, uint32_t) { ++cur[t][brick]; });
    });
    std::atomic<int> mismatch{0};
    run_threads(nt, [&](int t) {
        const int64_t pb = (nb + nt - 1) / nt, lo = std::min<int64_t>(nb, t * pb), hi = std::min<int64_t>(nb, lo + pb);
        for (int64_t b = lo; b < hi; ++b) {
            int64_t run = 0;
            for (int u = 0; u < nt; ++u) { const int32_t c = cur[u][b]; cur[u][b] = (int32_t)run; run += c; }
            if (run != brick_ptr[b + 1] - brick_ptr[b]) mismatch = 1;
        }
    });
    if (mismatch) return ig_fail(nullptr, IG_ERR_ARG, "ig_grid_shares_fill: brick_ptr does not come from ig_grid_shares_count");
    run_threads(nt, [&](int t) {
        int32_t* cursor = cur[t].data();
        const int64_t lo = std::min<int64_t>(M, t * per), hi = std::min<int64_t>(M, lo + per);
        for (int64_t s = lo; s < hi; ++s)
            for_shares(g, records + (size_t)s * g.rw, [&](int64_t brick, uint32_t geo, uint32_t gmask) {
                uint32_t* o = shares + 2 * (size_t)(brick_ptr[brick] + cursor[brick]++);
                o[0] = (uint32_t)s | (gmask << 28); o[1] = geo;
            });
    });
    return IG_OK;
}

int ig_grid_scatter_sep(ig_ctx* ctx, int64_t M, int64_t NC, int tw, void* records, int64_t rec_stride, const void* shares, const void* X, int64_t ldx,
                        void* Y_il, int64_t n0, int64_t nm, int64_t ns, int bm, int bs, const int32_t* tasks, int64_t ntasks,
                        const int32_t* brick_table, const int32_t* shared_table, int64_t nshared, int support_tile, float ar, float ai) {
    IG_REQUIRE(ctx, ctx != nullptr, "ig_grid_scatter_sep: ctx is NULL");
    ShareGeom g;
    IG_REQUIRE(ctx, M >= 0 && M < (1LL << 28) && (NC == 4 || NC == 8) && share_geom(g, tw, n0, nm, ns, bm, bs) && bm <= 4 && bs <= 4,
               "ig_grid_scatter_sep: 4 or 8 interleaved coils; a multiple of 16 points along x; bricks of 16 x (bm <= 4) x (bs <= 4) cells; tw 4, 6 or 8");
    IG_REQUIRE(ctx, support_tile == 16 || support_tile == 8 || support_tile == 4, "ig_grid_scatter_sep: support_tile 16, 8 or 4");
    IG_REQUIRE(ctx, ntasks >= 0 && ntasks <= 0x7fffffffLL && (ntasks == 0 || (tasks && brick_table && records && shares && X && Y_il)) && ldx >= M &&
               nshared >= 0 && (nshared == 0 || shared_table), "ig_grid_scatter_sep: bad task list or NULL array");
    IG_REQUIRE(ctx, n0 * nm * ns * (NC / 2) < (1LL << 32), "ig_grid_scatter_sep: grid panel too large");
    const int rw = sep_words(tw);
    IG_REQUIRE(ctx, rec_stride >= rw + 2 * NC && rec_stride % 4 == 0, "ig_grid_scatter_sep: record stride %lld words: the record (%d) and the panel row behind it", (long long)rec_stride, rw);
    if (ntasks == 0 || M == 0) return IG_OK;
    if (int rc = ig_set_device(ctx)) return rc;
    const float2 alpha = make_float2(ar, ai);
    int bm_log2 = 0, bs_log2 = 0;
    while ((1 << bm_log2) < bm) ++bm_log2;
    while ((1 << bs_log2) < bs) ++bs_log2;
    const int st_log2 = support_tile == 16 ? 4 : support_tile == 8 ? 3 : 2;
    const int nbx = (int)(n0 / 16), nbm = (int)((nm + bm - 1) / bm);
    const unsigned blocks = (unsigned)((ntasks + WPB - 1) / WPB);
    const size_t need = (size_t)M * NC * 8;
    int64_t gp = (M * NC + BLK - 1) / BLK;
    const int64_t cap = (int64_t)ctx->num_cu * 16;
    if (gp > cap) gp = cap;
#define IG_SM(NC_, TW_) do {                                                                                                             \
        {   ig_prof_scope prof(ctx, "pack_panel", 2.0 * (double)need);                                                                   \
            hipLaunchKernelGGL((k_sep_pack_recx<NC_>), dim3((unsigned)gp), dim3(BLK), 0, ctx->stream, M, (const float2*)X, ldx, (float2*)records, (int)(rec_stride / 2), rw / 2); } \
        if (nshared) {                                                                                                                   \
            ig_prof_scope prof(ctx, "grid_sep_zero");                                                                                    \
            hipLaunchKernelGGL((k_grid_sep_zero<NC_>), dim3((unsigned)nshared), dim3(BLK), 0, ctx->stream, (const ShareBrick*)shared_table, \
                               (float4*)Y_il, (int)n0, (int)nm, bm_log2, bs_log2, nbx, nbm, st_log2); }                                  \
        ig_prof_scope prof(ctx, "grid_scatter_sep");                                                                                     \
        hipLaunchKernelGGL((k_grid_scatter_mfma<NC_, TW_, 4>), dim3(blocks), dim3(BLK), 0, ctx->stream, (const ShareTask*)tasks, (int)ntasks, \
                           (const ShareBrick*)brick_table, (const uint2*)shares, (const uint32_t*)records, (int)rec_stride, (float*)Y_il, \
                           alpha, (int)n0, (int)nm, bm_log2, bs_log2, nbx, nbm, st_log2);                                                \
    } while (0)
#define IG_SM_TW(NC_) do { if (tw == 4) IG_SM(NC_, 4); else if (tw == 6) IG_SM(NC_, 6); else IG_SM(NC_, 8); } while (0)
    if (NC == 8) IG_SM_TW(8); else IG_SM_TW(4);
#undef IG_SM_TW
#undef IG_SM
    IG_LAUNCH_CHECK(ctx, "k_grid_scatter_mfma");
    return IG_OK;
}

}
```

indigo_amd/csrc/ig_spmm.hip:

```cpp
#include "ig_common.h"
#include <hip/amd_detail/amd_hip_unsafe_atomics.h>
#include <vector>
#include <thread>
#include <atomic>
#include <functional>
#include <algorithm>
#include <cstring>
#include <cstdlib>

namespace {

constexpr int BLK = 256;
constexpr int WAVES_PER_BLOCK = BLK / 64;

__device__ __forceinline__ int64_t xcd_block(int64_t b, int64_t nb) {
    const int64_t q = nb >> 3, rem = nb & 7;
    const int64_t xcd = b & 7, idx = b >> 3;
    return (xcd < rem) ? xcd * (q + 1) + idx : rem * (q + 1) + (xcd - rem) * q + idx;
}

struct GridMask {
    const uint32_t* bits;
    int64_t n0, nm;
};
// ... 2207 lines not shown
        if (rc[t] == 2) return ig_fail(nullptr, IG_ERR_UNSUPPORTED, "ig_grid_bricks_count: a row touches more than 64 bricks");
    }
    std::atomic<int> bad{0};
    run_threads(nt, [&](int t) {
        const int64_t pb = (g.nb + nt - 1) / nt, lo = std::min<int64_t>(g.nb, t * pb), hi = std::min<int64_t>(g.nb, lo + pb);
        for (int64_t b = lo; b < hi; ++b) {
            int64_t sum = 0;
            for (int u = 0; u < nt; ++u) sum += cnt[u][b];
            if (sum > 0x7fffffffLL) { bad = 1; sum = 0; }
            brick_entries[b] = (int32_t)sum;
        }
    });
    for (int t = 0; t < nt; ++t) if (ovf[t]) bad = 1;
    if (bad) return ig_fail(nullptr, IG_ERR_ARG, "ig_grid_bricks_count: a brick exceeds 2^31 entries");
    return IG_OK;
}

int ig_grid_bricks_fill(int64_t M, const int32_t* rowptr, const int32_t* colind, const void* vals, int64_t n0, int64_t nm, int64_t ns,
                        int bm, int bs, int unit, const int64_t* brick_ptr ,
                        void* entries ,
                        uint32_t* round_rows ) {
    if (M < 0 || !rowptr || !brick_ptr || !bricks_ok(n0, nm, ns, bm, bs, unit) || (rowptr[M] > rowptr[0] && (!colind || !vals || !entries || !round_rows)))
        return ig_fail(nullptr, IG_ERR_ARG, "ig_grid_bricks_fill: bad arguments");
    BrickGeom g{n0, nm, ns, n0 / 16, nm / bm, ns / bs, 0, bm, bs, unit};
    g.nb = g.nbx * g.nbm * g.nbs;
    const int64_t nbx = g.nbx, nbm = g.nbm;
    const int nt = brick_threads(M);
    const int64_t per = (M + nt - 1) / nt;
    std::vector<std::vector<int32_t>> cur((size_t)nt);
    std::vector<int> rc((size_t)nt, 0), ovf((size_t)nt, 0);
    run_threads(nt, [&](int t) {
        cur[t].assign((size_t)g.nb, 0);
        const int64_t lo = std::min<int64_t>(M, t * per), hi = std::min<int64_t>(M, lo + per);
        rc[t] = count_rows(g, rowptr, colind, lo, hi, cur[t].data(), &ovf[t]);
    });
    for (int t = 0; t < nt; ++t)
        if (rc[t] || ovf[t]) return ig_fail(nullptr, rc[t] == 2 ? IG_ERR_UNSUPPORTED : IG_ERR_ARG, "ig_grid_bricks_fill: the matrix does not fit the brick format (see ig_grid_bricks_count)");
    std::atomic<int> mismatch{0};
    run_threads(nt, [&](int t) {
        const int64_t pb = (g.nb + nt - 1) / nt, lo = std::min<int64_t>(g.nb, t * pb), hi = std::min<int64_t>(g.nb, lo + pb);
        for (int64_t b = lo; b < hi; ++b) {
            int64_t run = 0;
            for (int u = 0; u < nt; ++u) { const int32_t c = cur[u][b]; cur[u][b] = (int32_t)run; run += c; }
            if (run != brick_ptr[b + 1] - brick_ptr[b]) mismatch = 1;
        }
    });
    if (mismatch) return ig_fail(nullptr, IG_ERR_ARG, "ig_grid_bricks_fill: brick_ptr does not come from ig_grid_bricks_count");
    const float2* v = (const float2*)vals;
    BrickEntry* out = (BrickEntry*)entries;
    run_threads(nt, [&](int th) {
        int32_t* cursor = cur[th].data();
        const int64_t lo = std::min<int64_t>(M, th * per), hi = std::min<int64_t>(M, lo + per);
        for (int64_t t = lo; t < hi; ++t) {
            RowBricks rb;
            int64_t start[64];
            for (int32_t p = rowptr[t]; p < rowptr[t + 1]; ++p) {
                const int64_t col = colind[p];
                const int64_t kx = col % n0, km = (col / n0) % nm, ks = col / (n0 * nm);
                const int64_t b = kx / 16 + nbx * (km / bm + nbm * (ks / bs));
                const int before = rb.n;
                rb.add(b);
                int q = 0;
                while (rb.id[q] != b) ++q;
                if (rb.n > before) start[q] = brick_ptr[b] + cursor[b];
                BrickEntry e;
                e.cell = (uint32_t)((kx % 16) + 16 * ((km % bm) + bm * (ks % bs)));
                e.re = v[p].x; e.im = v[p].y;
                out[start[q] + rb.cnt[q] - 1] = e;
            }
            for (int q = 0; q < rb.n; ++q) {
                const int64_t padded = (rb.cnt[q] + unit - 1) / unit * unit;
                for (int64_t i = rb.cnt[q]; i < padded; ++i) {
                    BrickEntry e; e.cell = 0xffffffffu; e.re = 0.f; e.im = 0.f;
                    out[start[q] + i] = e;
                }
                for (int64_t i = 0; i < padded; i += unit) round_rows[(start[q] + i) / unit] = (uint32_t)t;
                cursor[rb.id[q]] += (int32_t)padded;
            }
        }
    });
    return IG_OK;
}

int ig_ccsrmm_t_bricks(ig_ctx* ctx, int64_t M, int64_t K, int64_t N, float ar, float ai,
                       const void* entries, const uint32_t* round_rows, const void* X, int64_t ldx, void* Y_il, const int16_t* support, int64_t n0, int64_t nm,
                       int bm, int bs, const int32_t* tasks, int64_t ntasks, const int32_t* brick_table,
                       const int32_t* shared_bricks, int64_t nshared, int support_tile, int support_zwords, int entry_words) {
    IG_REQUIRE(ctx, ctx != nullptr, "ig_ccsrmm_t_bricks: ctx is NULL");
    IG_REQUIRE(ctx, entry_words == 3 || entry_words == 2, "ig_ccsrmm_t_bricks: entries of 3 words {cell, re, im} or 2 {cell, re} (got %d)", entry_words);
    const bool realw = entry_words == 2;
    const int zw = support_zwords > 0 ? support_zwords : 16;
    IG_REQUIRE(ctx, M >= 0 && K >= 0 && M <= 0x7fffffffLL, "ig_ccsrmm_t_bricks: bad dimensions");
    IG_REQUIRE(ctx, N == 4 || N == 8, "ig_ccsrmm_t_bricks: 4 or 8 columns (got %lld); entries must be padded to 64/N per row and brick", (long long)N);
    IG_REQUIRE(ctx, (ntasks == 0 || (entries && round_rows)) && (M == 0 || X) && (K == 0 || Y_il) && ldx >= M, "ig_ccsrmm_t_bricks: NULL array or short leading dimension");
    IG_REQUIRE(ctx, n0 > 0 && nm > 0 && K % (n0 * nm) == 0 && K < 0x7fffffffLL && bricks_ok(n0, nm, K / (n0 * nm), bm, bs, 8) && bm * bs <= 32,
               "ig_ccsrmm_t_bricks: rows (%lld) are not a grid of n0=%lld x nm=%lld x ... that divides into 16 x %d x %d bricks", (long long)K, (long long)n0, (long long)nm, bm, bs);
    const int64_t ns = K / (n0 * nm);
    IG_REQUIRE(ctx, !support || (zw <= 64 && nm <= 32 * (int64_t)zw), "ig_ccsrmm_t_bricks: the support bitmaps hold 32 bits in each of %d words: nm <= %d", zw, 32 * zw);
    IG_REQUIRE(ctx, support_tile == 16 || support_tile == 8 || support_tile == 4, "ig_ccsrmm_t_bricks: support_tile %d (kx points per entry of the support table: 16, 8 or 4)", support_tile);
    IG_REQUIRE(ctx, (16 / support_tile) * bm * bs <= 32, "ig_ccsrmm_t_bricks: at most 32 segments per brick (%d x %d x %d)", 16 / support_tile, bm, bs);
    const int st_log2 = support_tile == 16 ? 4 : support_tile == 8 ? 3 : 2;
    IG_REQUIRE(ctx, ntasks >= 0 && ntasks <= 0x7fffffffLL && (ntasks == 0 || (tasks && brick_table)) && nshared >= 0 && (nshared == 0 || shared_bricks), "ig_ccsrmm_t_bricks: bad task list");
    IG_REQUIRE(ctx, M * N * 8 < 0x7fffffffLL, "ig_ccsrmm_t_bricks: the panel (%lld x %lld) exceeds the 2 GB window of a buffer descriptor", (long long)M, (long long)N);
    if (K == 0 || ntasks == 0) return IG_OK;
    if (int rc = ig_set_device(ctx)) return rc;
    const int64_t nt = n0 / 16;
    const int64_t snt = n0 / support_tile;
    const uint32_t* bits = support ? reinterpret_cast<const uint32_t*>(support + 2 * (ns * snt + snt)) : nullptr;
    const float2 alpha = make_float2(ar, ai);
    const size_t need = (size_t)M * N * 8;
    if (ctx->xpack_bytes < need) {
        if (ctx->d_xpack) { IG_HIP(ctx, hipStreamSynchronize(ctx->stream)); IG_HIP(ctx, hipFree(ctx->d_xpack)); ctx->d_xpack = nullptr; ctx->xpack_bytes = 0; }
        IG_HIP(ctx, hipMalloc((void**)&ctx->d_xpack, need));
        ctx->xpack_bytes = need;
    }
    float2* xp = (float2*)ctx->d_xpack;
    {
        ig_prof_scope prof(ctx, "pack_panel", 2.0 * (double)need);
        int64_t g = (M * N + BLK - 1) / BLK;
        const int64_t cap = (int64_t)ctx->num_cu * 16;
        if (g > cap) g = cap;
        if (N == 4) hipLaunchKernelGGL(k_pack_panel<4>, dim3((unsigned)g), dim3(BLK), 0, ctx->stream, M, N, (const float2*)X, ldx, xp, (const int32_t*)nullptr);
        else        hipLaunchKernelGGL(k_pack_panel<8>, dim3((unsigned)g), dim3(BLK), 0, ctx->stream, M, N, (const float2*)X, ldx, xp, (const int32_t*)nullptr);
        IG_LAUNCH_CHECK(ctx, "k_pack_panel");
    }
    int bm_log2 = 0, bs_log2 = 0;
    while ((1 << bm_log2) < bm) ++bm_log2;
    while ((1 << bs_log2) < bs) ++bs_log2;
    const int nbx = (int)nt, nbm = (int)(nm / bm);
    const size_t lds = (size_t)WAVES_PER_BLOCK * 16 * bm * bs * N * 8;
    IG_REQUIRE(ctx, lds <= 64 * 1024, "ig_ccsrmm_t_bricks: bricks of 16 x %d x %d points x %lld columns need %zu bytes of LDS per workgroup (limit 64 KB)", bm, bs, (long long)N, lds);
    const unsigned blocks = (unsigned)((ntasks + WAVES_PER_BLOCK - 1) / WAVES_PER_BLOCK);
#define IG_BRICKS(NC_, NSEG_) IG_BRICKS_P(NC_, NSEG_, false)
#define IG_BRICKS_P(NC_, NSEG_, PAIR_) do {                                                                                            \
        if (nshared) {                                                                                                          \
            ig_prof_scope prof(ctx, "grid_bricks_zero");                                                                        \
            hipLaunchKernelGGL((k_grid_bricks_zero<NC_>), dim3((unsigned)nshared), dim3(BLK), 0, ctx->stream, shared_bricks, (float2*)Y_il, bits, (int)n0, (int)nm, bm_log2, bs_log2, nbx, nbm, st_log2, zw); } \
        ig_prof_scope prof(ctx, "csrmm_bricks_conj");                                                                           \
        if (realw) hipLaunchKernelGGL((k_grid_bricks<NC_, NSEG_, PAIR_, true>), dim3(blocks), dim3(BLK), lds, ctx->stream, (const BrickTask*)tasks, (int)ntasks, (const BrickRef*)brick_table, (const BrickEntry*)entries, round_rows, \
                           (const float2*)xp, (float2*)Y_il, alpha, bits, (int)n0, (int)nm, bm_log2, bs_log2, nbx, nbm, st_log2, zw); \
        else hipLaunchKernelGGL((k_grid_bricks<NC_, NSEG_, PAIR_, false>), dim3(blocks), dim3(BLK), lds, ctx->stream, (const BrickTask*)tasks, (int)ntasks, (const BrickRef*)brick_table, (const BrickEntry*)entries, round_rows, \
                           (const float2*)xp, (float2*)Y_il, alpha, bits, (int)n0, (int)nm, bm_log2, bs_log2, nbx, nbm, st_log2, zw); } while (0)
    const int nseg_total = (16 / support_tile) * bm * bs;
    if (N == 8 && nseg_total == 4) IG_BRICKS(8, 4);
    else if (N == 8 && nseg_total == 8) IG_BRICKS(8, 8);
    else if (N == 8 && nseg_total == 16 && support_tile == 4) IG_BRICKS_P(8, 8, true);
    else if (N == 8) IG_BRICKS(8, 0);
    else IG_BRICKS(4, 0);
#undef IG_BRICKS
#undef IG_BRICKS_P
    IG_LAUNCH_CHECK(ctx, "k_grid_bricks");
    return IG_OK;
}

int ig_grid_slots_build(int64_t nbricks, const int64_t* brick_ptr, const void* entries12, const uint32_t* entry_rows, int ncell,
                        void* entries16, int32_t* brick_slots, int32_t* slot_ptr, int64_t* nslots) {
    if (nbricks < 0 || !brick_ptr || ncell < 1 || ncell > 1024 || !brick_slots || !slot_ptr || !nslots ||
        (brick_ptr[nbricks] > 0 && (!entries12 || !entry_rows || !entries16)) || brick_ptr[nbricks] > 0x7fffffffLL)
        return ig_fail(nullptr, IG_ERR_ARG, "ig_grid_slots_build: bad arguments");
    const BrickEntry* in = (const BrickEntry*)entries12;
    SlotEntry* out = (SlotEntry*)entries16;
    const int nt = brick_threads(nbricks * 8);
    const int64_t per = (nbricks + nt - 1) / nt;
    std::atomic<int> bad{0};
    run_threads(nt, [&](int th) {
        std::vector<int32_t> mult((size_t)ncell), gsize;
        const int64_t lo = std::min<int64_t>(nbricks, th * per), hi = std::min<int64_t>(nbricks, lo + per);
        for (int64_t b = lo; b < hi; ++b) {
            const int64_t p0 = brick_ptr[b], p1 = brick_ptr[b + 1];
            if (p1 == p0) { brick_slots[b] = 0; continue; }
            std::fill(mult.begin(), mult.end(), 0);
            gsize.clear();
            for (int64_t p = p0; p < p1; ++p) {
                const uint32_t c = in[p].cell;
                if (c >= (uint32_t)ncell) { bad = 1; continue; }
                const int k = mult[c]++;
                if ((size_t)k >= gsize.size()) gsize.push_back(0);
                ++gsize[k];
            }
            int64_t ns = 0;
            for (int32_t g : gsize) ns += (g + 63) / 64;
            brick_slots[b] = (int32_t)ns;
        }
    });
    if (bad) return ig_fail(nullptr, IG_ERR_ARG, "ig_grid_slots_build: a cell index outside the brick");
    std::vector<int64_t> first((size_t)nbricks + 1, 0);
    for (int64_t b = 0; b < nbricks; ++b) first[b + 1] = first[b] + brick_slots[b];
    if (first[nbricks] > 0x7fffffffLL) return ig_fail(nullptr, IG_ERR_ARG, "ig_grid_slots_build: more than 2^31 - 1 slots");
    *nslots = first[nbricks];
    run_threads(nt, [&](int th) {
        std::vector<int32_t> mult((size_t)ncell), gstart;
        std::vector<int32_t> gsize;
        const int64_t lo = std::min<int64_t>(nbricks, th * per), hi = std::min<int64_t>(nbricks, lo + per);
        for (int64_t b = lo; b < hi; ++b) {
            const int64_t p0 = brick_ptr[b], p1 = brick_ptr[b + 1];
            if (p1 == p0) continue;
            std::fill(mult.begin(), mult.end(), 0);
            gsize.clear();
            for (int64_t p = p0; p < p1; ++p) {
                const int k = mult[in[p].cell]++;
                if ((size_t)k >= gsize.size()) gsize.push_back(0);
                ++gsize[k];
            }
            gstart.assign(gsize.size() + 1, 0);
            for (size_t k = 0; k < gsize.size(); ++k) gstart[k + 1] = gstart[k] + gsize[k];
            int64_t s = first[b];
            for (size_t k = 0; k < gsize.size(); ++k)
                for (int32_t o = 0; o < gsize[k]; o += 64) slot_ptr[s++] = (int32_t)(p0 + gstart[k] + o);
            std::fill(mult.begin(), mult.end(), 0);
            std::vector<int32_t> cursor(gstart.begin(), gstart.end() - 1);
            for (int64_t p = p0; p < p1; ++p) {
                const int k = mult[in[p].cell]++;
                SlotEntry e; e.cell = in[p].cell; e.re = in[p].re; e.im = in[p].im; e.row = entry_rows[p];
                out[p0 + cursor[k]++] = e;
            }
        }
    });
    slot_ptr[first[nbricks]] = (int32_t)brick_ptr[nbricks];
    return IG_OK;
}

int ig_ccsrmm_t_slots(ig_ctx* ctx, int64_t M, int64_t K, int64_t N, float ar, float ai,
                      const void* entries16, const int32_t* slot_ptr, const void* X, int64_t ldx, void* Y_il, const int16_t* support,
                      int64_t n0, int64_t nm, int bm, int bs, const int32_t* tasks, int64_t ntasks, const int32_t* brick_table,
                      const int32_t* shared_bricks, int64_t nshared, int support_tile, int support_zwords, int entry_words) {
    IG_REQUIRE(ctx, ctx != nullptr, "ig_ccsrmm_t_slots: ctx is NULL");
    IG_REQUIRE(ctx, entry_words == 4 || entry_words == 3, "ig_ccsrmm_t_slots: entries of 4 words {cell, re, im, row} or 3 {cell, re, row} (got %d)", entry_words);
    const bool realw = entry_words == 3;
    const int zw = support_zwords > 0 ? support_zwords : 16;
    IG_REQUIRE(ctx, M >= 0 && K >= 0 && M <= 0x7fffffffLL, "ig_ccsrmm_t_slots: bad dimensions");
    IG_REQUIRE(ctx, N == 1 || N == 2 || N == 4, "ig_ccsrmm_t_slots: 1, 2 or 4 columns (got %lld; at 8 the round format of ig_ccsrmm_t_bricks is faster: 0.77 against 1.28 ms)", (long long)N);
    IG_REQUIRE(ctx, (ntasks == 0 || (entries16 && slot_ptr)) && (M == 0 || X) && (K == 0 || Y_il) && ldx >= M, "ig_ccsrmm_t_slots: NULL array or short leading dimension");
    IG_REQUIRE(ctx, n0 > 0 && nm > 0 && K % (n0 * nm) == 0 && K < 0x7fffffffLL && bricks_ok(n0, nm, K / (n0 * nm), bm, bs, 1) && bm * bs <= 32,
               "ig_ccsrmm_t_slots: rows (%lld) are not a grid of n0=%lld x nm=%lld x ... that divides into 16 x %d x %d bricks", (long long)K, (long long)n0, (long long)nm, bm, bs);
    const int64_t ns = K / (n0 * nm);
// ... 272 lines not shown
```

indigo_amd/dist.py:

```python
import ctypes
import hashlib
import os
import tempfile
import time

import numpy as np

_C64 = np.dtype('complex64')


def coil_range(C, rank, world):
    base, rem = divmod(C, world)
    lo = rank * base + min(rank, rem)
    return range(lo, lo + base + (1 if rank < rem else 0))


class _DevicePtr(object):

    def __init__(self, ptr, nfloats):
        self.__cuda_array_interface__ = dict(shape=(int(nfloats),), typestr='<f4', data=(int(ptr), False),
                                             version=2, strides=None)


def _rendezvous_path():
# ... 222 lines not shown

class TorchComm(object):
    overlap = False

    def __init__(self, backend):
        import torch
        import torch.distributed as dist
        assert dist.is_initialized(), "call torch.distributed.init_process_group first"
        self._torch, self._dist, self._backend = torch, dist, backend
        self.rank, self.world = dist.get_rank(), dist.get_world_size()
        self._on_gpu = hasattr(backend, 'stream')
        self._stream = None
        if self._on_gpu:
            self._device = torch.device('cuda', backend.device_id)
            self._stream = torch.cuda.ExternalStream(backend.stream, device=self._device)
        self._cache = {}

    def describe(self):
        return "torch.distributed (%s), %d ranks" % (self._dist.get_backend(), self.world)

    def _tensor(self, arr):
        assert arr.dtype == _C64 and arr.contiguous
        key = (id(arr._arr) if not self._on_gpu else arr._arr, arr.size)
        t = self._cache.get(key)
        if t is None:
            if self._on_gpu:
                t = self._torch.as_tensor(_DevicePtr(arr._arr, arr.size * 2), device=self._device)
            else:
                t = self._torch.from_numpy(arr._arr.reshape(-1, order='F').view(np.float32))
                assert t.data_ptr() == arr._arr.ctypes.data, "oracle array is not contiguous"
            self._cache = {key: t}
        return t

    def allreduce_(self, arr, force=False):
        if self.world == 1 and not force:
            return
        t = self._tensor(arr)
        if self._on_gpu:
            with self._torch.cuda.stream(self._stream):
                self._dist.all_reduce(t, op=self._dist.ReduceOp.SUM)
        else:
            self._dist.all_reduce(t, op=self._dist.ReduceOp.SUM)

    def join(self):
        pass

    def barrier(self):
        if self.world > 1:
            self._dist.barrier()

    def max(self, value):
        if self.world == 1:
            return value
        t = self._torch.tensor([value], dtype=self._torch.float64,
                               device=self._device if self._on_gpu else 'cpu')
        self._dist.all_reduce(t, op=self._dist.ReduceOp.MAX)
        return float(t.item())

    def allreduce(self, value):
        if self.world == 1:
            return value
        t = self._torch.tensor([value], dtype=self._torch.float64, device=self._device if self._on_gpu else 'cpu')
        self._dist.all_reduce(t, op=self._dist.ReduceOp.SUM)
        return float(t.item())

    def close(self):
        if self._dist.is_initialized():
            self._dist.destroy_process_group()


class ShardedNormalOperator(object):

    def __init__(self, A_local, comm, lamda=0.0, nslabs=4):
        self._A = A_local
        self._backend = A_local._backend
        self._comm = comm
        self._lamda = lamda
        n = A_local.shape[1]
        self.shape = (n, n)
        self.dtype = _C64
        self._ksp = None
        self._leaf = None
        self._nslabs = int(nslabs)
        self._route = 'undecided' if (getattr(comm, 'overlap', False) and comm.world > 1 and self._nslabs > 1) else 'full'
        if self._route == 'undecided':
            from indigo_amd import operators as op
            r = A_local
            if isinstance(r, op.VStack):
                r = r.children[-1]
            if isinstance(r, op.HeadRows):
                r = r.child
            while isinstance(r, op.Product):
                r = r.right
            if isinstance(r, op.ZpadFFT) and hasattr(self._backend, 'ifft_cropped_sum') and (r._layout == 2 or (r._layout == 1 and r._C == 1)):
                self._leaf = r

    def _covers(self, done):
        done = sorted(done)
        return bool(done) and done[0][0] == 0 and done[-1][1] == self.shape[1] and all(a[1] == b[0] for a, b in zip(done[:-1], done[1:]))

    def eval(self, y, x, alpha=1, beta=0, forward=True, left=True):
        assert alpha == 1 and beta == 0, "ShardedNormalOperator computes y = AHA x only"
        B = self._backend
        ncols = x.size // self.shape[1]
        if self._ksp is None or self._ksp.shape != (self._A.shape[0], ncols):
            self._ksp = B.zero_array((self._A.shape[0], ncols), _C64, name='ksp(shard)')
        self._A.eval(self._ksp, x)
        if self._route == 'undecided' and ncols == 1:
            done = []
            if self._leaf is not None:
                self._leaf._slab_hook = (self._nslabs, lambda arr, lo, hi: done.append((lo, hi)))
            try:
                self._A.eval(y, self._ksp, forward=False)
            finally:
                if self._leaf is not None:
                    self._leaf._slab_hook = None
            self._comm.allreduce_(y)
            cannot = 0.0 if self._covers(done) else 1.0
            self._route = 'slab' if self._comm.max(cannot) == 0.0 else 'full'
        elif self._route == 'slab' and ncols == 1:
            done = []

            def hook(arr, lo, hi):
                self._comm.allreduce_slab_(arr, lo, hi)
                done.append((lo, hi))
            self._leaf._slab_hook = (self._nslabs, hook)
            try:
                self._A.eval(y, self._ksp, forward=False)
            finally:
                self._leaf._slab_hook = None
            self._comm.join()
            if not self._covers(done):
                raise RuntimeError("slab all-reduce covered %s of [0, %d): the ranks' collectives no longer match" % (sorted(done), self.shape[1]))
        else:
            self._A.eval(y, self._ksp, forward=False)
            self._comm.allreduce_(y)
        if self._lamda:
            B.axpby(1, y, self._lamda, x)
```

indigo_amd/operators.py:

```python
import contextlib
import io
import numpy as np
import scipy.sparse as spp

_C64 = np.dtype('complex64')


def _is_number(v):
    return isinstance(v, (int, float, complex, np.number)) and not isinstance(v, bool)


class Operator(object):

    def __init__(self, backend, name='', alpha=1, batch=None):
        self._backend = backend
        self._name = name
        self._batch = batch

    def eval(self, y, x, alpha=1, beta=0, forward=True, left=True):
        if not left:
            raise NotImplementedError("Right-multiplication is not implemented for %s." % type(self).__name__)
        rows, cols = self.shape if forward else self.shape[::-1]
        x2 = x.reshape((cols, -1))
        y2 = y.reshape((rows, -1))
# ... 741 lines not shown

class DenseMatrix(Operator):

    def __init__(self, backend, M, **kwargs):
        super().__init__(backend, **kwargs)
        M = np.require(M, requirements='F')
        assert M.dtype == _C64 and M.ndim == 2
        self._matrix = M
        self._matrix_d = None

    @property
    def shape(self):
        return self._matrix.shape

    @property
    def dtype(self):
        return self._matrix.dtype

    def _eval(self, y, x, alpha=1, beta=0, forward=True, left=True):
        if self._matrix_d is None:
            self._matrix_d = self._backend.copy_array(self._matrix)
        self._backend.cgemm(y, self._matrix_d, x, alpha=alpha, beta=beta, forward=forward)



class Adjoint(CompositeOperator):
    def __init__(self, backend, child, *args, **kwargs):
        super().__init__(backend, child, *args, **kwargs)

    @property
    def shape(self):
        return self.child.shape[::-1]

    @property
    def dtype(self):
        return self.child.dtype

    @property
    def H(self):
        return self.child

    def _eval(self, y, x, alpha=1, beta=0, forward=True, left=True):
        self.child.eval(y, x, alpha, beta, forward=not forward, left=left)


class Scale(CompositeOperator):
    def __init__(self, backend, v, child, **kwargs):
        super().__init__(backend, child, **kwargs)
        self._name = "%s*{}".format(child._name)
        self._val = v

    @property
    def shape(self):
        return self.child.shape

    @property
    def dtype(self):
        return self.child.dtype

    def _eval(self, y, x, alpha=1, beta=0, forward=True, left=True):
        factor = self._val if forward else np.conj(self._val)
        self.child.eval(y, x, alpha=alpha * factor, beta=beta, forward=forward, left=left)


class Product(BinaryOperator):
    def __init__(self, *args, **kwargs):
        super().__init__(*args, **kwargs)
        self._name = "{}*{}".format(self.left._name, self.right._name)

    def _adopt(self, children):
        L, R = children
        if L.shape[1] != R.shape[0]:
            raise ValueError("Mismatched shapes in Product: attempting {} x {} ({} x {})".format(
                L.shape, R.shape, L._name, R._name))
        super()._adopt(children)

    @property
    def shape(self):
        return self.left.shape[0], self.right.shape[1]

    def _eval(self, y, x, alpha=1, beta=0, forward=True, left=True):
        L, R = self._children
        first, last = (R, L) if forward else (L, R)
        with self._backend.scratch(shape=(R.shape[0], x.shape[1])) as tmp:
            first.eval(tmp, x, alpha=alpha, beta=0, forward=forward, left=left)
            last.eval(y, tmp, alpha=1, beta=beta, forward=forward, left=left)

    def _mem_usage(self, ncols):
        ncols = min(ncols, self._batch or ncols)
        return self._children[1].shape[0] * ncols * self.dtype.itemsize


class Sum(BinaryOperator):
    def __init__(self, *args, **kwargs):
        super().__init__(*args, **kwargs)
        self._name = "{}+{}".format(self.left._name, self.right._name)

    def _adopt(self, children):
        L, R = children
        if L.shape != R.shape:
            raise ValueError("Mismatched shapes in Sum: attempting {} + {} ({} + {})".format(
                L.shape, R.shape, L._name, R._name))
        super()._adopt(children)

    @property
    def shape(self):
        return self.left.shape

    def _eval(self, y, x, alpha=1, beta=0, forward=True, left=True):
        L, R = self._children
        R.eval(y, x, alpha=alpha, beta=beta, forward=forward, left=left)
        L.eval(y, x, alpha=alpha, beta=1.0, forward=forward, left=left)


class Kron(BinaryOperator):

    @property
    def shape(self):
        h = int(np.prod([c.shape[0] for c in self._children]))
        w = int(np.prod([c.shape[1] for c in self._children]))
        return h, w

    def _eval(self, y, x, alpha=1, beta=0, forward=True, left=True):
        L, R = self._children
        if isinstance(L, Eye):
            if x.shape[1] > 1 and getattr(R, '_grid_interleaved', False):
                for j in range(x.shape[1]):
                    R.eval(y[:, j:j + 1], x[:, j:j + 1], alpha=alpha, beta=beta, forward=forward, left=left)
                return
            R.eval(y, x, alpha=alpha, beta=beta, forward=forward, left=left)
        else:
            raise NotImplementedError(
                "Kron with a non-identity left factor needs right-multiplication, which only the "
                "reference's dense real-symmetric path provides; outside the SENSE hot path.  For a temporal basis "
                "Phi (x) I_n use FrameBasis(phi, n).")


def _slice_rows(arr, start, stop):
    return arr[slice(start, stop), :]


class BlockDiag(CompositeOperator):
    @property
    def shape(self):
        return (sum(c.shape[0] for c in self._children), sum(c.shape[1] for c in self._children))

    def _eval(self, y, x, alpha=1, beta=0, forward=True, left=True):
        yo = xo = 0
        for C in self._children:
            h, w = C.shape if forward else C.shape[::-1]
            C.eval(y.dense_rows(yo, yo + h), x.dense_rows(xo, xo + w),
                   alpha=alpha, beta=beta, forward=forward, left=left)
            yo += h
            xo += w


class VStack(CompositeOperator):
    def _adopt(self, children):
        widths = [c.shape[1] for c in children]
        if len(set(widths)) > 1:
            raise ValueError("Mismatched widths in VStack: attempting to stack {}".format(
                list(zip(widths, [c._name for c in children]))))
        super()._adopt(children)

    @property
    def shape(self):
        return sum(c.shape[0] for c in self._children), self._children[-1].shape[1]

    def _eval(self, y, x, alpha=1, beta=0, forward=True, left=True):
        off = 0
        if forward:
            for C in self._children:
                h = C.shape[0]
                C.eval(_slice_rows(y, off, off + h), x, alpha=alpha, beta=beta, forward=True, left=left)
                off += h
        else:
            for i, C in enumerate(self._children):
                h = C.shape[0]
                C.eval(y, _slice_rows(x, off, off + h), alpha=alpha, beta=beta if i == 0 else 1, forward=False, left=left)
                off += h


class HeadRows(CompositeOperator):

    def __init__(self, backend, child, keep, **kwargs):
        super().__init__(backend, child, **kwargs)
        self._keep = int(keep)
        assert 0 < self._keep <= child.shape[0]

    @property
    def shape(self):
        return self._keep, self.child.shape[1]

    def _mem_usage(self, ncols):
        return self.child.shape[0] * ncols * 8
# ... 43 lines not shown
```

indigo_amd/sense.py:

```python
import numpy as np
import scipy.sparse as spp
from scipy.signal.windows import kaiser

from indigo_amd import fused
from indigo_amd import operators as op
from indigo_amd.interp import interp_csr_arrays, interp_csr_modulated, interp_sep_records
from indigo_amd.noncart import rolloff3
from indigo_amd.transforms import sense_recipe, reserve_for

_C64 = np.dtype('complex64')


def radial_trajectory(nspokes, nreadout, seed=3):
    rng = np.random.default_rng(seed)
    z = rng.uniform(-1.0, 1.0, nspokes)
    phi = rng.uniform(0.0, 2 * np.pi, nspokes)
    s = np.sqrt(1.0 - z * z)
    d = np.stack([s * np.cos(phi), s * np.sin(phi), z])
    t = (np.arange(nreadout) - nreadout // 2) / nreadout
    return d[:, None, :] * t[None, :, None]


class SenseProblem(object):

# ... 236 lines not shown
                           layout, chunks, table=table, row_order=order, zw=zw,
                           sep=self.fused_interp_sep(1, phases=folded) if (layout == 2 and order is None) else None, kshift=kshift)
        self.last_support_fine = getattr(A, '_support_fine', None)
        return A

    def build_zpadfft_maps(self, backend, maps, **kwargs):
        from indigo_amd.transforms import AttachCoilMaps
        maps = np.asarray(maps, dtype=_C64)
        assert maps.ndim == 5 and maps.shape[:3] == self.N, (maps.shape, self.N)
        if fused.image_permutation(backend, self.oN, int(maps.shape[3])) is not None:
            raise ValueError("build_zpadfft_maps: the fused leaf takes the grid %s only with its image axes permuted" % (self.oN,))
        ones = np.ones(self.N, dtype=_C64, order='F')
        q = SenseProblem(self.N, self.coord, lambda c: ones, width=self.width, ntable=self.ntable, oversamp=self.oversamp, ncoils=int(maps.shape[3]))
        q._interp_cache = self._interp_cache
        A = q.build_zpadfft(backend, **kwargs)
        for attr in ('last_support_table', 'last_support_zw', 'last_support_fine'):
            setattr(self, attr, getattr(q, attr, None))
        name = A._name
        A = AttachCoilMaps(maps).visit(A)
        A._name = name
        return A

    def permuted(self, perm):
        perm = tuple(int(a) for a in perm)
        N = tuple(self.N[a] for a in perm)
        if callable(self.maps):
            src = self.maps
            maps = (lambda c: src(c).transpose(perm))
        else:
            maps = self.maps.transpose(perm + (3,))
        q = SenseProblem(N, self.coord[list(perm)], maps, width=self.width, ntable=self.ntable, oversamp=self.oversamp, ncoils=self.C)
        assert q.oN == tuple(self.oN[a] for a in perm)
        q._interp_cache = self._interp_cache.setdefault(('permuted', perm), {})
        return q

    def build_fused(self, backend, coils=None):
        coils = list(range(self.C) if coils is None else coils)
        Cn = len(coils)
        G = backend.SpMatrix(self.fused_interp(), name='interp*mod*scale')
        F = backend.UnscaledFFT(self.oN, dtype=_C64, name='fft')
        St = backend.SpMatrix(self.fused_maps_T(coils), name='((x)mod*zpad*apod)*maps.H')
        A = backend.KronI(Cn, G) * (backend.KronI(Cn, F) * St.H)
        A._name = 'SENSE-O3'
        return A


def backend_mod(ft_shape):
    from indigo_amd.backends.backend import Backend
    return Backend.fftc_mod(ft_shape, _C64)


def _phases_key(phases):
    import hashlib
    h = hashlib.sha1()
    for ph in phases:
        a = np.ascontiguousarray(ph, dtype=np.float64)
        h.update(np.int64(a.size).tobytes())
        h.update(a.tobytes())
    return h.hexdigest()


def _mod_axis_phases(ft_shape):
    out = []
    for n in ft_shape:
        c = n // 2
        out.append((np.arange(n) - c / 2.0) * (c / n))
    return out


def fftc_mod_at(ft_shape, kx, ky, kz):
    px, py, pz = _mod_axis_phases(ft_shape)
    phase = 0 + px[kx]
    phase += py[ky]
    phase += pz[kz]
    return np.exp(1j * 2.0 * np.pi * phase).astype(_C64)


def fftc_mod_box(ft_shape, box):
    sl = [slice(m // 2 + int(np.ceil(-n / 2)), m // 2 + int(np.ceil(n / 2))) for m, n in zip(ft_shape, box)]
    ex, ey, ez = (np.exp(1j * 2.0 * np.pi * ph[s]) for ph, s in zip(_mod_axis_phases(ft_shape), sl))
    return np.asfortranarray((ex[:, None, None] * ey[None, :, None] * ez[None, None, :]).astype(_C64))


def normal_operator(A, lamda=0.0, ncols=1):
    AHA = A.H * A
    if lamda:
        AHA = lamda * A._backend.Eye(A.shape[1]) + AHA
    AHA._name = 'SENSE'
    reserve_for(AHA, ncols)
    return AHA
```

Measured before the change: 165.6.

## Fuse gridding normal operator with packed k-space handoff between gather and scatter

Adds a NormalGridding operator that evaluates K^H K as one unit, so the forward gridding gather writes k-space samples in a packed interleaved layout that the adjoint bricks or shares scatter reads directly. This skips the pack-panel step and the strided intermediate layout between the two halves. The Product wrapping it also evaluates in place, removing one scratch buffer for the FFT stage. It adds new entry points, an option flag, and an extra path that only triggers for single-column, contiguous, sep-route cases.

Result: no change. 167.7 (median of 6 runs) (+1.3%).

```diff
diff --git a/include/indigo_hip.h b/include/indigo_hip.h
--- a/include/indigo_hip.h
+++ b/include/indigo_hip.h
@@ -174,6 +174,11 @@
                         const int16_t* support, int64_t n0, int64_t nm, int bm, int bs, const int32_t* tasks, int64_t ntasks,
                         const int32_t* brick_table, const int32_t* shared_bricks, int64_t nshared, int support_tile, int support_zwords,
                         int entry_words);
+int  ig_ccsrmm_t_bricks_xp(ig_ctx* ctx, int64_t M, int64_t K, int64_t N, float alpha_re, float alpha_im,
+                           const void* entries, const uint32_t* round_rows, const void* Xp, void* Y_il,
+                           const int16_t* support, int64_t n0, int64_t nm, int bm, int bs, const int32_t* tasks, int64_t ntasks,
+                           const int32_t* brick_table, const int32_t* shared_bricks, int64_t nshared, int support_tile, int support_zwords,
+                           int entry_words);
 
 int  ig_grid_slots_build(int64_t nbricks, const int64_t* brick_ptr, const void* entries12, const uint32_t* entry_rows, int ncell,
                          void* entries16, int32_t* brick_slots, int32_t* slot_ptr, int64_t* nslots);
@@ -187,6 +192,8 @@
                         int64_t n0, int64_t nm, int64_t ns, float alpha_re, float alpha_im, float beta_re, float beta_im,
                         void* Y, int64_t ldy, const uint32_t* group_order);
 int  ig_grid_gather_sep_group(int64_t NC, int tw);
+int  ig_grid_gather_sep_packed(ig_ctx* ctx, int64_t M, int64_t NC, int tw, const void* records, int64_t rec_stride, const void* X_il,
+                               int64_t n0, int64_t nm, int64_t ns, float alpha_re, float alpha_im, void* Yp, const uint32_t* group_order);
 
 int  ig_grid_shares_count(int64_t M, const uint32_t* records, int tw, int64_t n0, int64_t nm, int64_t ns, int bm, int bs, int32_t* brick_shares);
 int  ig_grid_shares_fill(int64_t M, const uint32_t* records, int tw, int64_t n0, int64_t nm, int64_t ns, int bm, int bs,
@@ -195,6 +202,10 @@
                          void* Y_il, int64_t n0, int64_t nm, int64_t ns, int bm, int bs, const int32_t* tasks, int64_t ntasks,
                          const int32_t* brick_table, const int32_t* shared_table, int64_t nshared, int support_tile,
                          float alpha_re, float alpha_im);
+int  ig_grid_scatter_sep_xp(ig_ctx* ctx, int64_t M, int64_t NC, int tw, void* records, int64_t rec_stride, const void* shares, const void* Xp,
+                            void* Y_il, int64_t n0, int64_t nm, int64_t ns, int bm, int bs, const int32_t* tasks, int64_t ntasks,
+                            const int32_t* brick_table, const int32_t* shared_table, int64_t nshared, int support_tile,
+                            float alpha_re, float alpha_im);
 
 int  ig_ccsrmm_t_bricks_wide(ig_ctx* ctx, int64_t M, int64_t K, float alpha_re, float alpha_im,
                              const void* entries, const uint32_t* entry_rows, const void* X, int64_t ldx, void* Y, int64_t ldy,
diff --git a/indigo_amd/_lib.py b/indigo_amd/_lib.py
--- a/indigo_amd/_lib.py
+++ b/indigo_amd/_lib.py
@@ -99,6 +99,9 @@
     "ig_ccsrmm_t_bricks": (c_int, [c_void_p, c_int64, c_int64, c_int64, c_float, c_float, c_void_p, c_void_p,
                                    c_void_p, c_int64, c_void_p, c_void_p, c_int64, c_int64, c_int, c_int, c_void_p, c_int64,
                                    c_void_p, c_void_p, c_int64, c_int, c_int, c_int]),
+    "ig_ccsrmm_t_bricks_xp": (c_int, [c_void_p, c_int64, c_int64, c_int64, c_float, c_float, c_void_p, c_void_p,
+                                      c_void_p, c_void_p, c_void_p, c_int64, c_int64, c_int, c_int, c_void_p, c_int64,
+                                      c_void_p, c_void_p, c_int64, c_int, c_int, c_int]),
     "ig_ccsrmm":          (c_int, [c_void_p, c_int, c_int, c_int64, c_int64, c_int64, c_int64,
                                    c_float, c_float, c_void_p, c_void_p, c_void_p,
                                    c_void_p, c_int64, c_float, c_float, c_void_p, c_int64]),
@@ -149,10 +152,14 @@
     "ig_grid_gather_sep": (c_int, [c_void_p, c_int64, c_int64, c_int, c_void_p, c_int64, c_void_p, c_int64, c_int64, c_int64, c_float, c_float, c_float, c_float,
                                    c_void_p, c_int64, c_void_p]),
     "ig_grid_gather_sep_group": (c_int, [c_int64, c_int]),
+    "ig_grid_gather_sep_packed": (c_int, [c_void_p, c_int64, c_int64, c_int, c_void_p, c_int64, c_void_p, c_int64, c_int64, c_int64, c_float, c_float,
+                                          c_void_p, c_void_p]),
     "ig_grid_shares_count": (c_int, [c_int64, c_void_p, c_int, c_int64, c_int64, c_int64, c_int, c_int, c_void_p]),
     "ig_grid_shares_fill": (c_int, [c_int64, c_void_p, c_int, c_int64, c_int64, c_int64, c_int, c_int, c_void_p, c_void_p]),
     "ig_grid_scatter_sep": (c_int, [c_void_p, c_int64, c_int64, c_int, c_void_p, c_int64, c_void_p, c_void_p, c_int64, c_void_p, c_int64, c_int64, c_int64,
                                     c_int, c_int, c_void_p, c_int64, c_void_p, c_void_p, c_int64, c_int, c_float, c_float]),
+    "ig_grid_scatter_sep_xp": (c_int, [c_void_p, c_int64, c_int64, c_int, c_void_p, c_int64, c_void_p, c_void_p, c_void_p, c_int64, c_int64, c_int64,
+                                       c_int, c_int, c_void_p, c_int64, c_void_p, c_void_p, c_int64, c_int, c_float, c_float]),
     "ig_interp3_fill_modulated": (c_int, [c_int64, POINTER(c_int64), c_double, c_void_p, c_int64, c_void_p, c_void_p, c_void_p, c_void_p, c_int,
                                           c_void_p, c_void_p, c_void_p, c_double]),
     "ig_fft_plan":        (c_int, [c_void_p, c_int, POINTER(c_int64), c_int64, POINTER(c_void_p), POINTER(c_size_t)]),
diff --git a/indigo_amd/analyses.py b/indigo_amd/analyses.py
--- a/indigo_amd/analyses.py
+++ b/indigo_amd/analyses.py
@@ -36,7 +36,7 @@
         if isinstance(node, op.ZpadFFTMaps) and id(node) not in self._seen:
             self._seen.add(id(node))
             self._base += node.maps_bytes()
-        if isinstance(node, (op.Product, op.UnscaledFFT, op.ZpadFFT, op.HeadRows)):
+        if isinstance(node, (op.Product, op.NormalGridding, op.UnscaledFFT, op.ZpadFFT, op.HeadRows)):
             with self._push(self._live, self._round(node._mem_usage(self._ncols()))):
                 self._peak = max(self._peak, sum(self._live))
                 self.generic_visit(node)
diff --git a/indigo_amd/backends/backend.py b/indigo_amd/backends/backend.py
--- a/indigo_amd/backends/backend.py
+++ b/indigo_amd/backends/backend.py
@@ -260,6 +260,16 @@
             if n > 1e6:
                 log.info("  %40s: % 3.0f MB, %20s, %15s", name, n / 1e6, shape, dtype)
         return total
+
+    OPTIONS = {'grid.packed_handoff': 1}
+
+    def set_option(self, name, value):
+        if name not in self.OPTIONS:
+            raise ValueError("unknown option '%s'" % name)
+        self.__dict__.setdefault('_options', {})[name] = int(value)
+
+    def option(self, name):
+        return self.__dict__.get('_options', {}).get(name, self.OPTIONS[name])
 
     def reserve_scratch(self, nelems):
         self._scratch = self.empty_array((max(int(nelems), 1),), _C64, name='scratch')
@@ -311,6 +321,9 @@
 
     def Adjoint(self, A, **kwargs):
         return op.Adjoint(self, A, **kwargs)
+
+    def NormalGridding(self, K, **kwargs):
+        return op.NormalGridding(self, K, **kwargs)
 
     def KronI(self, c, B, **kwargs):
         return op.Kron(self, self.Eye(c), B, **kwargs)
@@ -774,6 +787,13 @@
             self._backend.ccsrmm(y, self.shape, self.colInds, self.rowPtrs, self.values,
                                  x, alpha=alpha, beta=beta, adjoint=True, exwrite=self._exwrite, **il)
 
+        def normal(self, y, x, alpha, tmp):
+            if not self._backend.option('grid.packed_handoff'):
+                return False
+            self.forward(tmp, x, alpha=alpha, beta=0)
+            self.adjoint(y, tmp, alpha=1, beta=0)
+            return True
+
         def set_grid_interleaved(self, flag=True):
             self._grid_il = bool(flag)
 
diff --git a/indigo_amd/backends/hip.py b/indigo_amd/backends/hip.py
--- a/indigo_amd/backends/hip.py
+++ b/indigo_amd/backends/hip.py
@@ -60,6 +60,8 @@
         return buf.value.decode()
 
     def set_option(self, name, value):
+        if name in self.OPTIONS:
+            return super().set_option(name, value)
         self._check(self._L.ig_set_option(self._ctx, name.encode(), int(value)), "ig_set_option(%s)" % name)
         for entry in self._plans.values():
             self._L.ig_fft_destroy(entry[0])
diff --git a/indigo_amd/backends/hip_csr.py b/indigo_amd/backends/hip_csr.py
--- a/indigo_amd/backends/hip_csr.py
+++ b/indigo_amd/backends/hip_csr.py
@@ -289,6 +289,35 @@
         self._check_panels(y, x, self.values)
         self._FORWARD[self.forward_route(x.shape[1])](self, y, x, alpha, beta)
 
+    def normal(self, y, x, alpha, tmp):
+        b, ncols = self._backend, x.shape[1]
+        if not (b.option('grid.packed_handoff') and self._grid_il and self._perm is None and x.contiguous and y.contiguous and tmp.contiguous
+                and tmp.size == self.shape[0] * ncols):
+            return False
+        if self.forward_route(ncols) != 'sep':
+            return False
+        route = self.adjoint_route(ncols, 0, y)
+        if route not in ('bricks', 'shares'):
+            return False
+        self._check_panels(y, x, self.values)
+        sep = self._sep
+        order = self._gather_order(ncols) if b.tuning.get('gather_order', True) else None
+        self._call("ig_grid_gather_sep_packed", self.shape[0], ncols, sep['tw'], sep['records']._arr, sep['stride'], x._arr, *sep['dims'],
+                   *_cplx(complex(alpha) * sep['gconst']), tmp._arr, _ptr(order))
+        if route == 'shares':
+            shf = self._format('_shares', ncols, exact=True)
+            self._scatter_support(ncols, y)
+            self._call("ig_grid_scatter_sep_xp", self.shape[0], ncols, sep['tw'], sep['recx']._arr, sep['stride_x'], shf['shares']._arr, tmp._arr,
+                       y._arr, *sep['dims'], shf['bm'], shf['bs'], shf['tasks']._arr, shf['ntasks'], shf['table']._arr,
+                       shf['shared']._arr, shf['nshared'], shf['tile'], *_cplx(np.conj(sep['gconst'])))
+        else:
+            f = self._format('_bricks', ncols, exact=True)
+            tab, tile = self._scatter_support(ncols, y)
+            self._call("ig_ccsrmm_t_bricks_xp", *self.shape, ncols, *_cplx(1), f['entries']._arr, f['rounds']._arr, tmp._arr, y._arr, _ptr(tab),
+                       f['n0'], f['nm'], f['bm'], f['bs'], f['tasks']._arr, f['ntasks'], f['table']._arr, f['shared']._arr, f['nshared'], tile,
+                       self._support_zw, f['words'])
+        return True
+
     def _adj_shares(self, y, x, alpha, beta):
         sep, shf = self._sep, self._format('_shares', x.shape[1], exact=True)
         self._scatter_support(x.shape[1], y)
diff --git a/indigo_amd/csrc/ig_gridsep.hip b/indigo_amd/csrc/ig_gridsep.hip
--- a/indigo_amd/csrc/ig_gridsep.hip
+++ b/indigo_amd/csrc/ig_gridsep.hip
@@ -51,7 +51,7 @@
 template <int NC, int TW, int BMODE>
 __global__ void __launch_bounds__(BLK)
 k_grid_gather_sep(int64_t M, const uint32_t* __restrict__ rec, int rs , const float4* __restrict__ X4, int n0, int nm, int ns,
-                  float2* __restrict__ Y, int64_t ldy, float2 alpha, float2 beta, const uint32_t* __restrict__ order) {
+                  float2* __restrict__ Y, int64_t ldy, float2 alpha, float2 beta, const uint32_t* __restrict__ order, int packed) {
     constexpr int QL = NC / 2, XL = TW <= 4 ? 4 : 8, LPS = QL * XL, SPW = 64 / LPS;
     constexpr int CG = TW <= 4 ? 4 : 2;
     static_assert(LPS <= 64 && NC >= 2, "a sample's lanes fit a wave");
@@ -94,12 +94,16 @@
         acc.z += __shfl_xor(acc.z, off, 64); acc.w += __shfl_xor(acc.w, off, 64);
     }
     if (i == 0 && ok) {
-        float2* y0 = Y + (int64_t)(2 * q) * ldy + t;
-        float2* y1 = y0 + ldy;
         float2 o0 = cmul(alpha, make_float2(acc.x, acc.y)), o1 = cmul(alpha, make_float2(acc.z, acc.w));
-        if (BMODE == 1) { cfma(o0, beta, *y0); cfma(o1, beta, *y1); }
-        *y0 = o0;
-        *y1 = o1;
+        if (BMODE == 0 && packed) {
+            reinterpret_cast<float4*>(Y)[t * QL + q] = make_float4(o0.x, o0.y, o1.x, o1.y);
+        } else {
+            float2* y0 = Y + (int64_t)(2 * q) * ldy + t;
+            float2* y1 = y0 + ldy;
+            if (BMODE == 1) { cfma(o0, beta, *y0); cfma(o1, beta, *y1); }
+            *y0 = o0;
+            *y1 = o1;
+        }
     }
 }
 
@@ -284,9 +288,9 @@
 
 template <int NC>
 __global__ void __launch_bounds__(BLK)
-k_sep_pack_recx(int64_t rows, const float2* __restrict__ X, int64_t ld, float2* __restrict__ recx2 , int rs2 , int rw2 ) {
+k_sep_pack_recx(int64_t rows, const float2* __restrict__ X, int64_t ld , float2* __restrict__ recx2 , int rs2 , int rw2 ) {
     for (int64_t e = (int64_t)blockIdx.x * BLK + threadIdx.x; e < rows * NC; e += (int64_t)gridDim.x * BLK)
-        recx2[(e / NC) * rs2 + rw2 + e % NC] = X[(e % NC) * ld + e / NC];
+        recx2[(e / NC) * rs2 + rw2 + e % NC] = ld ? X[(e % NC) * ld + e / NC] : X[e];
 }
 
 template <int NC>
@@ -382,13 +386,14 @@
     return WPB * (64 / ((int)(NC / 2) * (tw <= 4 ? 4 : 8)));
 }
 
-int ig_grid_gather_sep(ig_ctx* ctx, int64_t M, int64_t NC, int tw, const void* records, int64_t rec_stride, const void* X_il, int64_t n0, int64_t nm, int64_t ns,
-                       float ar, float ai, float br, float bi, void* Y, int64_t ldy, const uint32_t* group_order) {
+static int gather_sep(ig_ctx* ctx, int64_t M, int64_t NC, int tw, const void* records, int64_t rec_stride, const void* X_il, int64_t n0, int64_t nm, int64_t ns,
+                      float ar, float ai, float br, float bi, void* Y, int64_t ldy, const uint32_t* group_order, int packed) {
     IG_REQUIRE(ctx, ctx != nullptr, "ig_grid_gather_sep: ctx is NULL");
     IG_REQUIRE(ctx, M >= 0 && (NC == 2 || NC == 4 || NC == 8) && (tw == 4 || tw == 6 || tw == 8), "ig_grid_gather_sep: 2, 4 or 8 interleaved coils; tw 4, 6 or 8");
     IG_REQUIRE(ctx, n0 >= tw && nm >= tw && ns >= tw && n0 <= 65535 && nm <= 65535 && ns <= 65535 && n0 * nm * ns * (NC / 2) < (1LL << 32),
                "ig_grid_gather_sep: grid %lld x %lld x %lld x %lld coils out of range", (long long)n0, (long long)nm, (long long)ns, (long long)NC);
-    IG_REQUIRE(ctx, M == 0 || (records && X_il && Y && ldy >= M), "ig_grid_gather_sep: NULL pointer or ldy < M");
+    IG_REQUIRE(ctx, M == 0 || (records && X_il && Y && (packed || ldy >= M)), "ig_grid_gather_sep: NULL pointer or ldy < M");
+    IG_REQUIRE(ctx, !packed || ((reinterpret_cast<uintptr_t>(Y) & 15u) == 0 && br == 0.f && bi == 0.f), "ig_grid_gather_sep_packed: 16-byte aligned rows, beta = 0");
     IG_REQUIRE(ctx, rec_stride >= sep_words(tw) && rec_stride % 4 == 0 && rec_stride <= 1024, "ig_grid_gather_sep: record stride %lld words", (long long)rec_stride);
     IG_REQUIRE(ctx, (reinterpret_cast<uintptr_t>(X_il) & 15u) == 0 && (reinterpret_cast<uintptr_t>(records) & 15u) == 0, "ig_grid_gather_sep: 16-byte aligned panel and records");
     if (M == 0) return IG_OK;
@@ -401,9 +406,9 @@
         const int64_t blocks = ((M + spw - 1) / spw + WPB - 1) / WPB;                                                            \
         IG_REQUIRE(ctx, blocks <= 0x7fffffffLL, "ig_grid_gather_sep: too many samples for one launch");                          \
         if (b0) hipLaunchKernelGGL((k_grid_gather_sep<NC_, TW_, 0>), dim3((unsigned)blocks), dim3(BLK), 0, ctx->stream, M,       \
-                                   (const uint32_t*)records, (int)rec_stride, (const float4*)X_il, (int)n0, (int)nm, (int)ns, (float2*)Y, ldy, alpha, beta, group_order); \
+                                   (const uint32_t*)records, (int)rec_stride, (const float4*)X_il, (int)n0, (int)nm, (int)ns, (float2*)Y, ldy, alpha, beta, group_order, packed); \
         else    hipLaunchKernelGGL((k_grid_gather_sep<NC_, TW_, 1>), dim3((unsigned)blocks), dim3(BLK), 0, ctx->stream, M,       \
-                                   (const uint32_t*)records, (int)rec_stride, (const float4*)X_il, (int)n0, (int)nm, (int)ns, (float2*)Y, ldy, alpha, beta, group_order); \
+                                   (const uint32_t*)records, (int)rec_stride, (const float4*)X_il, (int)n0, (int)nm, (int)ns, (float2*)Y, ldy, alpha, beta, group_order, packed); \
     } while (0)
 #define IG_GS_TW(NC_) do { if (tw == 4) IG_GS(NC_, 4); else if (tw == 6) IG_GS(NC_, 6); else IG_GS(NC_, 8); } while (0)
     if (NC == 8) IG_GS_TW(8);
@@ -413,6 +418,16 @@
 #undef IG_GS
     IG_LAUNCH_CHECK(ctx, "k_grid_gather_sep");
     return IG_OK;
+}
+
+int ig_grid_gather_sep(ig_ctx* ctx, int64_t M, int64_t NC, int tw, const void* records, int64_t rec_stride, const void* X_il, int64_t n0, int64_t nm, int64_t ns,
+                       float ar, float ai, float br, float bi, void* Y, int64_t ldy, const uint32_t* group_order) {
+    return gather_sep(ctx, M, NC, tw, records, rec_stride, X_il, n0, nm, ns, ar, ai, br, bi, Y, ldy, group_order, 0);
+}
+
+int ig_grid_gather_sep_packed(ig_ctx* ctx, int64_t M, int64_t NC, int tw, const void* records, int64_t rec_stride, const void* X_il, int64_t n0, int64_t nm, int64_t ns,
+                              float ar, float ai, void* Yp, const uint32_t* group_order) {
+    return gather_sep(ctx, M, NC, tw, records, rec_stride, X_il, n0, nm, ns, ar, ai, 0.f, 0.f, Yp, 0, group_order, 1);
 }
 
 
@@ -481,15 +496,15 @@
     return IG_OK;
 }
 
-int ig_grid_scatter_sep(ig_ctx* ctx, int64_t M, int64_t NC, int tw, void* records, int64_t rec_stride, const void* shares, const void* X, int64_t ldx,
-                        void* Y_il, int64_t n0, int64_t nm, int64_t ns, int bm, int bs, const int32_t* tasks, int64_t ntasks,
-                        const int32_t* brick_table, const int32_t* shared_table, int64_t nshared, int support_tile, float ar, float ai) {
+static int scatter_sep(ig_ctx* ctx, int64_t M, int64_t NC, int tw, void* records, int64_t rec_stride, const void* shares, const void* X, int64_t ldx, bool rows,
+                       void* Y_il, int64_t n0, int64_t nm, int64_t ns, int bm, int bs, const int32_t* tasks, int64_t ntasks,
+                       const int32_t* brick_table, const int32_t* shared_table, int64_t nshared, int support_tile, float ar, float ai) {
     IG_REQUIRE(ctx, ctx != nullptr, "ig_grid_scatter_sep: ctx is NULL");
     ShareGeom g;
     IG_REQUIRE(ctx, M >= 0 && M < (1LL << 28) && (NC == 4 || NC == 8) && share_geom(g, tw, n0, nm, ns, bm, bs) && bm <= 4 && bs <= 4,
                "ig_grid_scatter_sep: 4 or 8 interleaved coils; a multiple of 16 points along x; bricks of 16 x (bm <= 4) x (bs <= 4) cells; tw 4, 6 or 8");
     IG_REQUIRE(ctx, support_tile == 16 || support_tile == 8 || support_tile == 4, "ig_grid_scatter_sep: support_tile 16, 8 or 4");
-    IG_REQUIRE(ctx, ntasks >= 0 && ntasks <= 0x7fffffffLL && (ntasks == 0 || (tasks && brick_table && records && shares && X && Y_il)) && ldx >= M &&
+    IG_REQUIRE(ctx, ntasks >= 0 && ntasks <= 0x7fffffffLL && (ntasks == 0 || (tasks && brick_table && records && shares && X && Y_il)) && (rows || ldx >= M) &&
                nshared >= 0 && (nshared == 0 || shared_table), "ig_grid_scatter_sep: bad task list or NULL array");
     IG_REQUIRE(ctx, n0 * nm * ns * (NC / 2) < (1LL << 32), "ig_grid_scatter_sep: grid panel too large");
     const int rw = sep_words(tw);
@@ -508,8 +523,8 @@
     const int64_t cap = (int64_t)ctx->num_cu * 16;
     if (gp > cap) gp = cap;
 #define IG_SM(NC_, TW_) do {                                                                                                             \
-        {   ig_prof_scope prof(ctx, "pack_panel", 2.0 * (double)need);                                                                   \
-            hipLaunchKernelGGL((k_sep_pack_recx<NC_>), dim3((unsigned)gp), dim3(BLK), 0, ctx->stream, M, (const float2*)X, ldx, (float2*)records, (int)(rec_stride / 2), rw / 2); } \
+        {   ig_prof_scope prof(ctx, rows ? "panel_rows" : "pack_panel", 2.0 * (double)need);                                             \
+            hipLaunchKernelGGL((k_sep_pack_recx<NC_>), dim3((unsigned)gp), dim3(BLK), 0, ctx->stream, M, (const float2*)X, rows ? (int64_t)0 : ldx, (float2*)records, (int)(rec_stride / 2), rw / 2); } \
         if (nshared) {                                                                                                                   \
             ig_prof_scope prof(ctx, "grid_sep_zero");                                                                                    \
             hipLaunchKernelGGL((k_grid_sep_zero<NC_>), dim3((unsigned)nshared), dim3(BLK), 0, ctx->stream, (const ShareBrick*)shared_table, \
@@ -527,4 +542,18 @@
     return IG_OK;
 }
 
-}
+int ig_grid_scatter_sep(ig_ctx* ctx, int64_t M, int64_t NC, int tw, void* records, int64_t rec_stride, const void* shares, const void* X, int64_t ldx,
+                        void* Y_il, int64_t n0, int64_t nm, int64_t ns, int bm, int bs, const int32_t* tasks, int64_t ntasks,
+                        const int32_t* brick_table, const int32_t* shared_table, int64_t nshared, int support_tile, float ar, float ai) {
+    return scatter_sep(ctx, M, NC, tw, records, rec_stride, shares, X, ldx, false, Y_il, n0, nm, ns, bm, bs, tasks, ntasks, brick_table, shared_table, nshared,
+                       support_tile, ar, ai);
+}
+
+int ig_grid_scatter_sep_xp(ig_ctx* ctx, int64_t M, int64_t NC, int tw, void* records, int64_t rec_stride, const void* shares, const void* Xp,
+                           void* Y_il, int64_t n0, int64_t nm, int64_t ns, int bm, int bs, const int32_t* tasks, int64_t ntasks,
+                           const int32_t* brick_table, const int32_t* shared_table, int64_t nshared, int support_tile, float ar, float ai) {
+    return scatter_sep(ctx, M, NC, tw, records, rec_stride, shares, Xp, 0, true, Y_il, n0, nm, ns, bm, bs, tasks, ntasks, brick_table, shared_table, nshared,
+                       support_tile, ar, ai);
+}
+
+}
diff --git a/indigo_amd/csrc/ig_spmm.hip b/indigo_amd/csrc/ig_spmm.hip
--- a/indigo_amd/csrc/ig_spmm.hip
+++ b/indigo_amd/csrc/ig_spmm.hip
@@ -2313,17 +2313,17 @@
     return IG_OK;
 }
 
-int ig_ccsrmm_t_bricks(ig_ctx* ctx, int64_t M, int64_t K, int64_t N, float ar, float ai,
-                       const void* entries, const uint32_t* round_rows, const void* X, int64_t ldx, void* Y_il, const int16_t* support, int64_t n0, int64_t nm,
-                       int bm, int bs, const int32_t* tasks, int64_t ntasks, const int32_t* brick_table,
-                       const int32_t* shared_bricks, int64_t nshared, int support_tile, int support_zwords, int entry_words) {
+static int ccsrmm_t_bricks(ig_ctx* ctx, int64_t M, int64_t K, int64_t N, float ar, float ai,
+                           const void* entries, const uint32_t* round_rows, const void* X, int64_t ldx, const void* Xp, void* Y_il, const int16_t* support, int64_t n0, int64_t nm,
+                           int bm, int bs, const int32_t* tasks, int64_t ntasks, const int32_t* brick_table,
+                           const int32_t* shared_bricks, int64_t nshared, int support_tile, int support_zwords, int entry_words) {
     IG_REQUIRE(ctx, ctx != nullptr, "ig_ccsrmm_t_bricks: ctx is NULL");
     IG_REQUIRE(ctx, entry_words == 3 || entry_words == 2, "ig_ccsrmm_t_bricks: entries of 3 words {cell, re, im} or 2 {cell, re} (got %d)", entry_words);
     const bool realw = entry_words == 2;
     const int zw = support_zwords > 0 ? support_zwords : 16;
     IG_REQUIRE(ctx, M >= 0 && K >= 0 && M <= 0x7fffffffLL, "ig_ccsrmm_t_bricks: bad dimensions");
     IG_REQUIRE(ctx, N == 4 || N == 8, "ig_ccsrmm_t_bricks: 4 or 8 columns (got %lld); entries must be padded to 64/N per row and brick", (long long)N);
-    IG_REQUIRE(ctx, (ntasks == 0 || (entries && round_rows)) && (M == 0 || X) && (K == 0 || Y_il) && ldx >= M, "ig_ccsrmm_t_bricks: NULL array or short leading dimension");
+    IG_REQUIRE(ctx, (ntasks == 0 || (entries && round_rows)) && (M == 0 || X || Xp) && (K == 0 || Y_il) && (Xp || ldx >= M), "ig_ccsrmm_t_bricks: NULL array or short leading dimension");
     IG_REQUIRE(ctx, n0 > 0 && nm > 0 && K % (n0 * nm) == 0 && K < 0x7fffffffLL && bricks_ok(n0, nm, K / (n0 * nm), bm, bs, 8) && bm * bs <= 32,
                "ig_ccsrmm_t_bricks: rows (%lld) are not a grid of n0=%lld x nm=%lld x ... that divides into 16 x %d x %d bricks", (long long)K, (long long)n0, (long long)nm, bm, bs);
     const int64_t ns = K / (n0 * nm);
@@ -2339,21 +2339,23 @@
     const int64_t snt = n0 / support_tile;
     const uint32_t* bits = support ? reinterpret_cast<const uint32_t*>(support + 2 * (ns * snt + snt)) : nullptr;
     const float2 alpha = make_float2(ar, ai);
-    const size_t need = (size_t)M * N * 8;
-    if (ctx->xpack_bytes < need) {
-        if (ctx->d_xpack) { IG_HIP(ctx, hipStreamSynchronize(ctx->stream)); IG_HIP(ctx, hipFree(ctx->d_xpack)); ctx->d_xpack = nullptr; ctx->xpack_bytes = 0; }
-        IG_HIP(ctx, hipMalloc((void**)&ctx->d_xpack, need));
-        ctx->xpack_bytes = need;
-    }
-    float2* xp = (float2*)ctx->d_xpack;
-    {
+    const float2* xp = (const float2*)Xp;
+    if (!xp) {
+        const size_t need = (size_t)M * N * 8;
+        if (ctx->xpack_bytes < need) {
+            if (ctx->d_xpack) { IG_HIP(ctx, hipStreamSynchronize(ctx->stream)); IG_HIP(ctx, hipFree(ctx->d_xpack)); ctx->d_xpack = nullptr; ctx->xpack_bytes = 0; }
+            IG_HIP(ctx, hipMalloc((void**)&ctx->d_xpack, need));
+            ctx->xpack_bytes = need;
+        }
+        float2* xw = (float2*)ctx->d_xpack;
         ig_prof_scope prof(ctx, "pack_panel", 2.0 * (double)need);
         int64_t g = (M * N + BLK - 1) / BLK;
         const int64_t cap = (int64_t)ctx->num_cu * 16;
         if (g > cap) g = cap;
-        if (N == 4) hipLaunchKernelGGL(k_pack_panel<4>, dim3((unsigned)g), dim3(BLK), 0, ctx->stream, M, N, (const float2*)X, ldx, xp, (const int32_t*)nullptr);
-        else        hipLaunchKernelGGL(k_pack_panel<8>, dim3((unsigned)g), dim3(BLK), 0, ctx->stream, M, N, (const float2*)X, ldx, xp, (const int32_t*)nullptr);
+        if (N == 4) hipLaunchKernelGGL(k_pack_panel<4>, dim3((unsigned)g), dim3(BLK), 0, ctx->stream, M, N, (const float2*)X, ldx, xw, (const int32_t*)nullptr);
+        else        hipLaunchKernelGGL(k_pack_panel<8>, dim3((unsigned)g), dim3(BLK), 0, ctx->stream, M, N, (const float2*)X, ldx, xw, (const int32_t*)nullptr);
         IG_LAUNCH_CHECK(ctx, "k_pack_panel");
+        xp = xw;
     }
     int bm_log2 = 0, bs_log2 = 0;
     while ((1 << bm_log2) < bm) ++bm_log2;
@@ -2382,6 +2384,23 @@
 #undef IG_BRICKS_P
     IG_LAUNCH_CHECK(ctx, "k_grid_bricks");
     return IG_OK;
+}
+
+int ig_ccsrmm_t_bricks(ig_ctx* ctx, int64_t M, int64_t K, int64_t N, float ar, float ai,
+                       const void* entries, const uint32_t* round_rows, const void* X, int64_t ldx, void* Y_il, const int16_t* support, int64_t n0, int64_t nm,
+                       int bm, int bs, const int32_t* tasks, int64_t ntasks, const int32_t* brick_table,
+                       const int32_t* shared_bricks, int64_t nshared, int support_tile, int support_zwords, int entry_words) {
+    return ccsrmm_t_bricks(ctx, M, K, N, ar, ai, entries, round_rows, X, ldx, nullptr, Y_il, support, n0, nm, bm, bs, tasks, ntasks, brick_table,
+                           shared_bricks, nshared, support_tile, support_zwords, entry_words);
+}
+
+int ig_ccsrmm_t_bricks_xp(ig_ctx* ctx, int64_t M, int64_t K, int64_t N, float ar, float ai,
+                          const void* entries, const uint32_t* round_rows, const void* Xp, void* Y_il, const int16_t* support, int64_t n0, int64_t nm,
+                          int bm, int bs, const int32_t* tasks, int64_t ntasks, const int32_t* brick_table,
+                          const int32_t* shared_bricks, int64_t nshared, int support_tile, int support_zwords, int entry_words) {
+    IG_REQUIRE(ctx, ctx == nullptr || M == 0 || (Xp && (reinterpret_cast<uintptr_t>(Xp) & 15u) == 0), "ig_ccsrmm_t_bricks_xp: NULL or misaligned packed panel");
+    return ccsrmm_t_bricks(ctx, M, K, N, ar, ai, entries, round_rows, nullptr, 0, Xp, Y_il, support, n0, nm, bm, bs, tasks, ntasks, brick_table,
+                           shared_bricks, nshared, support_tile, support_zwords, entry_words);
 }
 
 int ig_grid_slots_build(int64_t nbricks, const int64_t* brick_ptr, const void* entries12, const uint32_t* entry_rows, int ncell,
diff --git a/indigo_amd/dist.py b/indigo_amd/dist.py
--- a/indigo_amd/dist.py
+++ b/indigo_amd/dist.py
@@ -328,6 +328,11 @@
         self._ksp = None
         self._leaf = None
         self._nslabs = int(nslabs)
+        from indigo_amd.sense import gridding_normal_form
+        from indigo_amd.transforms import reserve_for
+        self._normal = gridding_normal_form(A_local)
+        if self._normal is not None:
+            reserve_for(self._normal, 1)
         self._route = 'undecided' if (getattr(comm, 'overlap', False) and comm.world > 1 and self._nslabs > 1) else 'full'
         if self._route == 'undecided':
             from indigo_amd import operators as op
@@ -349,15 +354,22 @@
         assert alpha == 1 and beta == 0, "ShardedNormalOperator computes y = AHA x only"
         B = self._backend
         ncols = x.size // self.shape[1]
-        if self._ksp is None or self._ksp.shape != (self._A.shape[0], ncols):
-            self._ksp = B.zero_array((self._A.shape[0], ncols), _C64, name='ksp(shard)')
-        self._A.eval(self._ksp, x)
+        if self._normal is not None and ncols == 1:
+            def adjoint():
+                self._normal.eval(y, x)
+        else:
+            if self._ksp is None or self._ksp.shape != (self._A.shape[0], ncols):
+                self._ksp = B.zero_array((self._A.shape[0], ncols), _C64, name='ksp(shard)')
+            self._A.eval(self._ksp, x)
+
+            def adjoint():
+                self._A.eval(y, self._ksp, forward=False)
         if self._route == 'undecided' and ncols == 1:
             done = []
             if self._leaf is not None:
                 self._leaf._slab_hook = (self._nslabs, lambda arr, lo, hi: done.append((lo, hi)))
             try:
-                self._A.eval(y, self._ksp, forward=False)
+                adjoint()
             finally:
                 if self._leaf is not None:
                     self._leaf._slab_hook = None
@@ -372,14 +384,14 @@
                 done.append((lo, hi))
             self._leaf._slab_hook = (self._nslabs, hook)
             try:
-                self._A.eval(y, self._ksp, forward=False)
+                adjoint()
             finally:
                 self._leaf._slab_hook = None
             self._comm.join()
             if not self._covers(done):
                 raise RuntimeError("slab all-reduce covered %s of [0, %d): the ranks' collectives no longer match" % (sorted(done), self.shape[1]))
         else:
-            self._A.eval(y, self._ksp, forward=False)
+            adjoint()
             self._comm.allreduce_(y)
         if self._lamda:
             B.axpby(1, y, self._lamda, x)
diff --git a/indigo_amd/operators.py b/indigo_amd/operators.py
--- a/indigo_amd/operators.py
+++ b/indigo_amd/operators.py
@@ -847,11 +847,20 @@
     def _eval(self, y, x, alpha=1, beta=0, forward=True, left=True):
         L, R = self._children
         first, last = (R, L) if forward else (L, R)
+        if forward and beta == 0 and self._in_place():
+            R.eval(y, x, alpha=alpha, beta=0, forward=True, left=left)
+            L.eval(y, y, alpha=1, beta=0, forward=True, left=left)
+            return
         with self._backend.scratch(shape=(R.shape[0], x.shape[1])) as tmp:
             first.eval(tmp, x, alpha=alpha, beta=0, forward=forward, left=left)
             last.eval(y, tmp, alpha=1, beta=beta, forward=forward, left=left)
 
+    def _in_place(self):
+        return isinstance(self._children[0], NormalGridding)
+
     def _mem_usage(self, ncols):
+        if self._in_place():
+            return 0
         ncols = min(ncols, self._batch or ncols)
         return self._children[1].shape[0] * ncols * self.dtype.itemsize
 
@@ -876,6 +885,43 @@
         L, R = self._children
         R.eval(y, x, alpha=alpha, beta=beta, forward=forward, left=left)
         L.eval(y, x, alpha=alpha, beta=1.0, forward=forward, left=left)
+
+
+class NormalGridding(CompositeOperator):
+
+    def __init__(self, backend, K, **kwargs):
+        assert isinstance(K, Kron) and isinstance(K.left, Eye) and isinstance(K.right, SpMatrix), "NormalGridding: K = KronI(c, SpMatrix)"
+        super().__init__(backend, K, **kwargs)
+        self._name = "{}.H*{}".format(K._name, K._name)
+
+    @property
+    def shape(self):
+        return (self.child.shape[1],) * 2
+
+    @property
+    def H(self):
+        return self
+
+    def _mem_usage(self, ncols):
+        return self.child.shape[0] * ncols * self.dtype.itemsize
+
+    def _eval(self, y, x, alpha=1, beta=0, forward=True, left=True):
+        K = self.child
+        G, c = K.right, K.left.shape[0]
+        if not forward:
+            alpha = np.conj(alpha)
+        with self._backend.scratch(shape=(K.shape[0], x.shape[1])) as tmp:
+            if beta == 0 and x.shape[1] == 1:
+                M = G._get_or_create_device_matrix()
+                xg, yg, tg = x.reshape((G.shape[1], c)), y.reshape((G.shape[1], c)), tmp.reshape((G.shape[0], c))
+                if hasattr(M, 'normal') and M.normal(yg, xg, alpha, tg):
+                    trace = getattr(self._backend, 'trace', None)
+                    if trace is not None:
+                        for xs, ys, fwd in ((xg, tg, True), (tg, yg, False)):
+                            trace.add('csrmm', nbytes=G.csrmm_bytes(xs, ys, 0, fwd), nflops=5 * G.nnz * c, shape=xs.shape, forward=fwd, name=G._name)
+                    return
+            K.eval(tmp, x, alpha=alpha, beta=0, forward=True, left=left)
+            K.eval(y, tmp, alpha=1, beta=beta, forward=False, left=left)
 
 
 class Kron(BinaryOperator):
diff --git a/indigo_amd/sense.py b/indigo_amd/sense.py
--- a/indigo_amd/sense.py
+++ b/indigo_amd/sense.py
@@ -342,8 +342,23 @@
     return np.asfortranarray((ex[:, None, None] * ey[None, :, None] * ez[None, None, :]).astype(_C64))
 
 
+def gridding_normal_form(A):
+    from indigo_amd import operators as op
+    if type(A) is op.HeadRows:
+        A = A.child
+    if not (type(A) is op.Product and isinstance(A.right, op.ZpadFFT)):
+        return None
+    K, Z = A.left, A.right
+    if not (type(K) is op.Kron and isinstance(K.left, op.Eye) and type(K.right) is op.SpMatrix):
+        return None
+    B = A._backend
+    return Z.H * (B.NormalGridding(K) * Z)
+
+
 def normal_operator(A, lamda=0.0, ncols=1):
-    AHA = A.H * A
+    AHA = gridding_normal_form(A)
+    if AHA is None:
+        AHA = A.H * A
     if lamda:
         AHA = lamda * A._backend.Eye(A.shape[1]) + AHA
     AHA._name = 'SENSE'
```
